# yyNoBug/VAE_segmentation

Hardware: AMD Instinct MI355X
Metric: 3D train-step volumes/sec at 96^3 batch=2 (joint VAE+seg) (higher is better)
Workload: dtype bf16; 1 GPU; configs[1]: 96^3 joint VAE+seg training step (joint_train), batch=2/GPU, bf16 activations + fp32 accumulate, SGD momentum 0.9, VAE frozen, HIP-graph replay; global_batch=2, parallelism=dp1, activation_recomputation=False, tail_in_graph=True, nranks=1, grad_exchange=none (1 rank)

## Files before the change

vae_segmentation_amd/csrc/conv_api.hip:

```cpp
#include <stdlib.h>
#include "igemm_dispatch.h"

int g1_dispatch_k3_f32(const G1Params& p, int ck, int mt, int epi, int tiles, int row_tiles, hipStream_t s);
int g1_dispatch_k3_bf16(const G1Params& p, int ck, int mt, int epi, int tiles, int row_tiles, hipStream_t s);
int g1_dispatch_k3_f16(const G1Params& p, int ck, int mt, int epi, int tiles, int row_tiles, hipStream_t s);
int g1_k3_fa_supported(const G1Params& p, int ck, int mt);
int k3tw_slab_count(int n, int d, int h, int w);
int k3x_ea_capacity(int n, int c, int m);
int k3b_ea_capacity(int n, int c, int m);
int k2s2_scatter8_launch(const G1Params& p, int dtype, hipStream_t stream);
int g1_dispatch_k3_x3(const G1Params& p, int ck, int mt, int epi, int tiles, int row_tiles, hipStream_t s);

extern "C" int vs_conv_k3_f32_limbs(int d, int h, int w, int c_in) {
    const int on = vs_cfg().f32_limbs;
    if (!on) return 0;
    const int small = vs_cfg().k3_small;
    if (small && c_in % 32 == 0 && c_in <= 1024 && (long long)(d + 2) * (h + 2) * (w + 2) <= 512) return 0;
    return 1;
}

static int dispatch_k3(const G1Params& p, int dtype, int ck, int mt, int epi, int tiles, int row_tiles, hipStream_t s) {
    if (dtype == VS_F32 && vs_conv_k3_f32_limbs(p.D, p.H, p.W, p.C)) {
        G1Params q = p;
        const int ckx = vs_k3x_ck(p.C);
        q.nch = p.C / ckx;
        const int rows16 = epi == EPI_SOFTMAX2 ? 16 : p.rb_total * 16;
        int mtx = 16;
        if (rows16 % 32 == 0 && (long long)tiles * (rows16 / 32) >= 256 && (ckx == 8 || (size_t)2 * p.N * (p.C + p.M) * sizeof(float) <= 3000)) mtx = 32;
        return g1_dispatch_k3_x3(q, ckx, mtx, epi, tiles, rows16 / mtx, s);
    }
    if (dtype == VS_F32) return g1_dispatch_k3_f32(p, ck, mt, epi, tiles, row_tiles, s);
    if (dtype == VS_BF16) return g1_dispatch_k3_bf16(p, ck, mt, epi, tiles, row_tiles, s);
    return g1_dispatch_k3_f16(p, ck, mt, epi, tiles, row_tiles, s);
}

static int pick_mt(int rows16, long long tiles) {
    const int min_wgs = vs_cfg().mt_min_wgs;
    const int cands[3] = {64, 32, 16};
    for (int i = 0; i < 3; ++i) {
        const int mt = cands[i];
        if (rows16 % mt) continue;
        if (tiles * (rows16 / mt) >= min_wgs || mt == 16) return mt;
    }
    return 16;
}

static int check_common(const void* x, const void* w, int n, int d, int h, int w_, int c_in, int dtype) {
    if (!x || !w) return VS_EINVAL;
    if (n <= 0 || d <= 0 || h <= 0 || w_ <= 0) return VS_ESHAPE;
    if (!(c_in == 8 || c_in == 16 || (c_in % 32 == 0 && c_in > 0 && c_in <= 256))) return VS_ESHAPE;
    if (!vs_dtype_ok(dtype)) return VS_EDTYPE;
    if (((uintptr_t)x & 15) || ((uintptr_t)w & 15)) return VS_EALIGN;
    if ((double)n * d * h * w_ * c_in >= 2147483648.0) return VS_ESHAPE;
    return VS_OK;
}

static inline long long g1_ea_capacity() { return 256; }

static int gather_impl(const void* x, const double* x_stats, const void* w_packed, const float* bias,
                       void* y, double* y_stats, const void* mask_x, const double* mask_stats, double* sums,
                       int n, int d, int h, int w, int c_in, int m_out, int kind, int dtype, float eps, void* stream,
                       const void* fa_x = nullptr, const double* fa_sums = nullptr, void* fa_dx = nullptr, int* fa_query = nullptr, float* wg_ws = nullptr,
                       unsigned int* ea_sync = nullptr, unsigned int* ea_fault = nullptr, int* ea_query = nullptr, const void* ea_add = nullptr) {
    int rc = check_common(x, w_packed, n, d, h, w, c_in, dtype);
    if (rc) return rc;
    if (!y || m_out <= 0 || m_out % 8 || ((uintptr_t)y & 15)) return VS_EINVAL;
    if (kind != VS_CONV_K3 && kind != VS_CONV_K2S2) return VS_EINVAL;
    if (kind == VS_CONV_K2S2 && ((d | h | w) & 1)) return VS_ESHAPE;
    G1Params p{};
    p.x = x; p.x_stats = x_stats; p.wp = w_packed; p.bias = bias; p.y = y; p.y_stats = y_stats; p.prob = nullptr;
    p.mask_x = mask_x; p.mask_stats = mask_stats; p.sums = sums;
    p.fa_x = fa_x; p.fa_sums = fa_sums; p.fa_dx = fa_dx; p.wg_ws = wg_ws;
    p.ea_sync = ea_sync; p.ea_fault = ea_fault; p.ea_add = ea_add;
    if (sums && (!mask_x || !mask_stats || y_stats)) return VS_EINVAL;
    p.N = n; p.D = d; p.H = h; p.W = w;
    p.C = c_in; p.M = m_out;
    p.rb_total = (m_out + 15) / 16;
    const int ck = c_in < 32 ? c_in : 32;
    p.nch = c_in / ck;
    p.eps = eps;
    p.inv_count_in = 1.0 / ((double)d * h * w);
    long long tiles;
    if (kind == VS_CONV_K3) {
        p.Do = d; p.Ho = h; p.Wo = w;
        p.tyn = (h + 3) / 4; p.txn = (w + 15) / 16;
        p.tiles_per_sample = ((d + 3) / 4) * p.tyn * p.txn;
    } else {
        p.Do = d / 2; p.Ho = h / 2; p.Wo = w / 2;
        p.tyn = p.txn = 0;
        p.tiles_per_sample = vs_ceil_div((long long)p.Do * p.Ho * p.Wo, 256);
        if (ck == 32 && p.nch >= 2 && (long long)p.tiles_per_sample * n * p.rb_total <= 64) {
            p.tiles_per_sample = vs_ceil_div((long long)p.Do * p.Ho * p.Wo, 64);
            p.tyn = 64;
        }
    }
    tiles = (long long)p.tiles_per_sample * n;
    p.inv_count_out = 1.0 / ((double)p.Do * p.Ho * p.Wo);
    const int rows16 = p.rb_total * 16;
    int mt = (kind != VS_CONV_K3 && p.tyn == 64) ? 16 : pick_mt(rows16, tiles);
    if (kind == VS_CONV_K3 && fa_x != nullptr && ck == 32 && mt == 16 && rows16 % 32 == 0) mt = 32;
    const int row_tiles = rows16 / mt;
    if (kind == VS_CONV_K2S2 && (ea_query != nullptr || ea_sync != nullptr)) {
        const bool ok = sums != nullptr && mt == 16 && tiles * row_tiles <= g1_ea_capacity();
        if (ea_query != nullptr) { *ea_query = ok ? 1 : 0; return VS_OK; }
        if (!ok) return VS_ESHAPE;
        p.ea_items = p.tiles_per_sample * row_tiles;
    }
    if (ea_query != nullptr) {
        *ea_query = (kind == VS_CONV_K3 && dtype != VS_F32 && ck == 32 && mt == 16 && sums != nullptr && !fa_x &&
                     !((long long)(d + 2) * (h + 2) * (w + 2) <= 512 && c_in <= 1024) && tiles * row_tiles <= k3b_ea_capacity(n, c_in, m_out)) ? 1 : 0;
        if (kind == VS_CONV_K3 && dtype == VS_F32 && sums != nullptr && !fa_x && vs_conv_k3_f32_limbs(d, h, w, c_in) && vs_k3x_ck(c_in) == 8 && c_in > 8) {
            const long long rows16 = p.rb_total;
            const bool mt32 = (p.rb_total * 16) % 32 == 0 && tiles * (p.rb_total / 2) >= 256;
            *ea_query = (!mt32 && tiles * rows16 <= k3x_ea_capacity(n, c_in, m_out)) ? 1 : 0;
        }
        return VS_OK;
    }
    if (fa_query != nullptr) {
        if (dtype == VS_F32)
            *fa_query = kind == VS_CONV_K3 && vs_conv_k3_f32_limbs(d, h, w, c_in) &&
                        ((c_in == 8 && m_out == 8 && n * 8 <= 192 && vs_k3x_toeplitz(8, 8, 27)) ||
                         (c_in == 16 && m_out == 16 && n * 16 <= 192 && vs_k3x_ck(16) == 8));
        else
            *fa_query = kind == VS_CONV_K3 ? g1_k3_fa_supported(p, ck, mt) : 0;
        return VS_OK;
    }
    if (kind == VS_CONV_K3) {
        return dispatch_k3(p, dtype, ck, mt, EPI_RAW, (int)tiles, row_tiles, (hipStream_t)stream);
    }
    return g1_dispatch_k2s2(p, dtype, ck, mt, (int)tiles, row_tiles, (hipStream_t)stream);
}

extern "C" int vs_conv_gather_fwd(const void* x, const double* x_stats, const void* w_packed, const float* bias,
                                  void* y, double* y_stats, int n, int d, int h, int w, int c_in, int m_out,
                                  int kind, int dtype, float eps, void* stream) {
    return gather_impl(x, x_stats, w_packed, bias, y, y_stats, nullptr, nullptr, nullptr, n, d, h, w, c_in, m_out, kind, dtype, eps, stream);
}

extern "C" int vs_conv_gather_bwd_data(const void* x, const void* w_packed, void* y, const void* mask_x,
                                       const double* mask_stats, double* sums, int n, int d, int h, int w, int c_in,
                                       int m_out, int kind, int dtype, float eps, void* stream) {
    if (!mask_x || !mask_stats || !sums) return VS_EINVAL;
    return gather_impl(x, nullptr, w_packed, nullptr, y, nullptr, mask_x, mask_stats, sums, n, d, h, w, c_in, m_out, kind, dtype, eps, stream);
}

extern "C" int vs_conv_k3_bwd_data_fused_apply(const void* g, const void* act_x, const double* act_stats, const double* act_sums,
                                               const void* w_packed, void* y, const void* mask_x, const double* mask_stats, double* sums,
                                               void* dx_out, int n, int d, int h, int w, int c_in, int m_out, int dtype, float eps,
                                               void* stream) {
    if (!g || !act_x || !act_stats || !act_sums) return VS_EINVAL;
    if ((mask_x == nullptr) != (sums == nullptr) || (mask_x == nullptr) != (mask_stats == nullptr)) return VS_EINVAL;
    if (dtype == VS_F32 && !vs_conv_k3_fused_apply_supported(n, d, h, w, c_in, m_out, mask_x != nullptr, dtype)) return VS_ESHAPE;
    if (((uintptr_t)act_x & 15) || (dx_out && ((uintptr_t)dx_out & 15))) return VS_EALIGN;
    return gather_impl(g, act_stats, w_packed, nullptr, y, nullptr, mask_x, mask_stats, sums, n, d, h, w, c_in, m_out, VS_CONV_K3, dtype, eps,
                       stream, act_x, act_sums, dx_out);
}

extern "C" int vs_conv_k3_fused_apply_supported(int n, int d, int h, int w, int c_in, int m_out, int lazy_input, int dtype) {
    if (!vs_dtype_ok(dtype)) return 0;
    static const char dummy[16] __attribute__((aligned(16))) = {0};
    static double dsink[2];
    int ok = 0;
    const int rc = gather_impl(dummy, (const double*)dummy, dummy, nullptr, (void*)dummy, nullptr, lazy_input ? dummy : nullptr,
                               lazy_input ? (const double*)dummy : nullptr, lazy_input ? dsink : nullptr, n, d, h, w, c_in, m_out, VS_CONV_K3,
                               dtype, 1e-5f, nullptr, dummy, (const double*)dummy, nullptr, &ok);
    return rc == VS_OK ? ok : 0;
}

extern "C" int vs_conv_k3_bwd_data_applied_supported(int n, int d, int h, int w, int c_in, int m_out, int dtype) {
    const int on = vs_cfg().epilogue_apply;
    if (!on || !vs_dtype_ok(dtype)) return 0;
    static const char dummy[16] __attribute__((aligned(16))) = {0};
    static double dsink[2];
    int ok = 0;
    const int rc = gather_impl(dummy, nullptr, dummy, nullptr, (void*)dummy, nullptr, dummy, (const double*)dummy, dsink, n, d, h, w, c_in, m_out, VS_CONV_K3, dtype,
                               1e-5f, nullptr, nullptr, nullptr, nullptr, nullptr, nullptr, nullptr, nullptr, &ok);
    return rc == VS_OK ? ok : 0;
}

extern "C" int vs_conv_k3_bwd_data_applied(const void* x, const void* w_packed, void* y, const void* mask_x, const double* mask_stats, double* sums,
                                           unsigned int* sync, unsigned int* fault, int n, int d, int h, int w, int c_in, int m_out, int dtype, float eps, void* stream) {
    if (!mask_x || !mask_stats || !sums || !sync || !fault) return VS_EINVAL;
    if (((uintptr_t)sync & 127) || ((uintptr_t)fault & 3)) return VS_EALIGN;
    if (!vs_conv_k3_bwd_data_applied_supported(n, d, h, w, c_in, m_out, dtype)) return VS_ESHAPE;
    return gather_impl(x, nullptr, w_packed, nullptr, y, nullptr, mask_x, mask_stats, sums, n, d, h, w, c_in, m_out, VS_CONV_K3, dtype, eps, stream,
                       nullptr, nullptr, nullptr, nullptr, nullptr, sync, fault);
}

extern "C" int vs_conv_k3_bwd_data_wgrad_supported(int n, int d, int h, int w, int c_in, int m_out, int dtype) {
    const int on = vs_cfg().fuse_wgrad;
    if (!on || (dtype != VS_BF16 && dtype != VS_F16)) return 0;
    if (c_in != 8 || m_out != 8 || n <= 0 || n * 8 > 192 || d <= 0 || h <= 0 || w <= 0) return 0;
    if ((double)n * d * h * w * 16 >= 2147483648.0) return 0;
    return vs_k3_toeplitz(8, 8, 27, dtype) ? 1 : 0;
}

extern "C" int vs_conv_k3_bwd_data_wgrad_slabs(int n, int d, int h, int w) {
    if (n <= 0 || d <= 0 || h <= 0 || w <= 0) return 0;
    return k3tw_slab_count(n, d, h, w);
}

extern "C" int vs_conv_k3_bwd_data_wgrad(const void* g, const void* act_x, const double* act_stats, const double* act_sums, const void* w_packed, void* y,
                                         const void* mask_x, const double* mask_stats, double* sums, float* slabs, int n, int d, int h, int w, int c_in,
                                         int m_out, int dtype, float eps, void* stream) {
    if (!g || !slabs || !mask_x || !mask_stats || !sums) return VS_EINVAL;
    if ((act_x == nullptr) != (act_stats == nullptr) || (act_x == nullptr) != (act_sums == nullptr)) return VS_EINVAL;
    if (!vs_conv_k3_bwd_data_wgrad_supported(n, d, h, w, c_in, m_out, dtype)) return VS_ESHAPE;
    if (((uintptr_t)slabs & 15) || (act_x && ((uintptr_t)act_x & 15))) return VS_EALIGN;
    return gather_impl(g, act_stats, w_packed, nullptr, y, nullptr, mask_x, mask_stats, sums, n, d, h, w, c_in, m_out, VS_CONV_K3, dtype, eps,
                       stream, act_x, act_sums, nullptr, nullptr, slabs);
}

extern "C" int vs_conv_k3_softmax2_bwd_data(const float* prob, const float* gprob, const void* gprob_cl, const void* w_packed, void* y, const void* mask_x,
                                            const double* mask_stats, double* sums, float* slabs, double* bias_part, int n, int d, int h, int w, int dtype,
                                            float eps, float drop_p, unsigned long long drop_seed, void* stream) {
    if (!prob || (!gprob && !gprob_cl) || !w_packed || !y || !mask_x || !mask_stats || !sums) return VS_EINVAL;
    if (bias_part && !slabs) return VS_EINVAL;
    if (!vs_conv_k3_bwd_data_wgrad_supported(n, d, h, w, 8, 8, dtype)) return VS_ESHAPE;
    if (((uintptr_t)w_packed & 15) || ((uintptr_t)y & 15) || ((uintptr_t)mask_x & 15) || (gprob_cl && ((uintptr_t)gprob_cl & 15)) || (slabs && ((uintptr_t)slabs & 15)) ||
        ((uintptr_t)prob & 3) || ((uintptr_t)gprob & 3)) return VS_EALIGN;
    if (!(drop_p >= 0.f && drop_p < 1.f)) return VS_EINVAL;
    G1Params p{};
    p.wp = w_packed; p.y = y; p.mask_x = mask_x; p.mask_stats = mask_stats; p.sums = sums;
    p.sm_prob = prob; p.sm_gprob = gprob; p.sm_gcl = gprob_cl; p.wg_ws = slabs; p.wg_bias = bias_part;
    p.drop_p = drop_p; p.drop_seed = drop_seed;
    p.N = n; p.D = d; p.H = h; p.W = w; p.Do = d; p.Ho = h; p.Wo = w; p.C = 8; p.M = 8; p.rb_total = 1; p.nch = 1;
    p.eps = eps;
    p.inv_count_in = 1.0 / ((double)d * h * w); p.inv_count_out = p.inv_count_in;
    return dispatch_k3(p, dtype, 8, 16, EPI_RAW, 0, 1, (hipStream_t)stream);
}

static int scatter_impl(const void* x, const double* x_stats, const void* w_packed, const float* bias, void* y,
                        const void* mask_x, const double* mask_stats, double* sums, int n, int d, int h, int w, int c_in,
                        int m_out, int dtype, float eps, void* stream,
                        unsigned int* ea_sync = nullptr, unsigned int* ea_fault = nullptr, int* ea_query = nullptr, const void* ea_add = nullptr) {
    int rc = check_common(x, w_packed, n, d, h, w, c_in, dtype);
    if (rc) return rc;
    if (!y || m_out <= 0 || m_out % 8 || ((uintptr_t)y & 15)) return VS_EINVAL;
    G1Params p{};
    p.x = x; p.x_stats = x_stats; p.wp = w_packed; p.bias = bias; p.y = y; p.y_stats = nullptr; p.prob = nullptr;
    p.mask_x = mask_x; p.mask_stats = mask_stats; p.sums = sums;
    p.inv_count_out = 1.0 / (8.0 * d * h * w);
    p.N = n; p.D = d; p.H = h; p.W = w;
    p.Do = d; p.Ho = h; p.Wo = w;
    p.C = c_in; p.M = m_out;
    p.rb_total = (8 * m_out + 15) / 16;
    const int ck = c_in < 32 ? c_in : 32;
    p.nch = c_in / ck;
    p.eps = eps;
    p.inv_count_in = 1.0 / ((double)d * h * w);
    p.tiles_per_sample = vs_ceil_div((long long)d * h * w, 256);
    const long long tiles = (long long)p.tiles_per_sample * n;
    const int stream8 = vs_cfg().k2s2_stream;
    const bool ea_asked = ea_query != nullptr || ea_sync != nullptr;
    if (!ea_asked && stream8 && sums && c_in == 8 && m_out == 8 && dtype != VS_F32 && !bias && !x_stats) {
        rc = k2s2_scatter8_launch(p, dtype, (hipStream_t)stream);
        if (rc != VS_ESHAPE) return rc;
    }
    const int rows16 = p.rb_total * 16;
    const int mt = pick_mt(rows16, tiles);
    if (ea_asked) {
        const bool ok = sums != nullptr && mt == 16 && tiles * (rows16 / mt) <= g1_ea_capacity();
        if (ea_query != nullptr) { *ea_query = ok ? 1 : 0; return VS_OK; }
        if (!ok) return VS_ESHAPE;
        p.ea_sync = ea_sync; p.ea_fault = ea_fault; p.ea_add = ea_add;
        p.ea_items = p.tiles_per_sample * (rows16 / mt);
    }
    return g1_dispatch_pw(p, dtype, ck, mt, (int)tiles, rows16 / mt, (hipStream_t)stream);
}

extern "C" int vs_conv_scatter_fwd(const void* x, const double* x_stats, const void* w_packed, const float* bias,
                                   void* y, int n, int d, int h, int w, int c_in, int m_out, int dtype, float eps,
                                   void* stream) {
    return scatter_impl(x, x_stats, w_packed, bias, y, nullptr, nullptr, nullptr, n, d, h, w, c_in, m_out, dtype, eps, stream);
}

extern "C" int vs_conv_scatter_bwd_data(const void* x, const void* w_packed, void* y, const void* mask_x,
                                        const double* mask_stats, double* sums, int n, int d, int h, int w, int c_in,
                                        int m_out, int dtype, float eps, void* stream) {
    if (!mask_x || !mask_stats || !sums) return VS_EINVAL;
    return scatter_impl(x, nullptr, w_packed, nullptr, y, mask_x, mask_stats, sums, n, d, h, w, c_in, m_out, dtype, eps, stream);
}

extern "C" int vs_conv_s2_bwd_data_applied_supported(int n, int d, int h, int w, int c_in, int m_out, int scatter, int dtype) {
    const int on = vs_cfg().epilogue_apply;
    if (!on || !vs_dtype_ok(dtype)) return 0;
    static const char dummy[16] __attribute__((aligned(16))) = {0};
    static double dsink[2];
    int ok = 0;
    const int rc = scatter ? scatter_impl(dummy, nullptr, dummy, nullptr, (void*)dummy, dummy, (const double*)dummy, dsink, n, d, h, w, c_in, m_out, dtype, 1e-5f, nullptr,
                                          nullptr, nullptr, &ok)
                           : gather_impl(dummy, nullptr, dummy, nullptr, (void*)dummy, nullptr, dummy, (const double*)dummy, dsink, n, d, h, w, c_in, m_out, VS_CONV_K2S2, dtype,
                                         1e-5f, nullptr, nullptr, nullptr, nullptr, nullptr, nullptr, nullptr, nullptr, &ok);
    return rc == VS_OK ? ok : 0;
}

extern "C" int vs_conv_s2_bwd_data_applied(const void* x, const void* w_packed, void* y, const void* mask_x, const double* mask_stats, double* sums, const void* add,
                                           unsigned int* sync, unsigned int* fault, int n, int d, int h, int w, int c_in, int m_out, int scatter, int dtype, float eps,
                                           void* stream) {
    if (!mask_x || !mask_stats || !sums || !sync || !fault) return VS_EINVAL;
    if (((uintptr_t)sync & 127) || ((uintptr_t)fault & 3) || (add && ((uintptr_t)add & 15))) return VS_EALIGN;
    if (!vs_conv_s2_bwd_data_applied_supported(n, d, h, w, c_in, m_out, scatter, dtype)) return VS_ESHAPE;
    if (scatter) return scatter_impl(x, nullptr, w_packed, nullptr, y, mask_x, mask_stats, sums, n, d, h, w, c_in, m_out, dtype, eps, stream, sync, fault, nullptr, add);
    return gather_impl(x, nullptr, w_packed, nullptr, y, nullptr, mask_x, mask_stats, sums, n, d, h, w, c_in, m_out, VS_CONV_K2S2, dtype, eps, stream,
                       nullptr, nullptr, nullptr, nullptr, nullptr, sync, fault, nullptr, add);
}

extern "C" int vs_conv_k3_softmax2_fwd(const void* x, const double* x_stats, const void* w_packed, const float* bias,
                                       float* prob, int n, int d, int h, int w, int c_in, int dtype, float eps,
                                       void* stream) {
    return vs_conv_k3_softmax2_dropout_fwd(x, x_stats, w_packed, bias, prob, n, d, h, w, c_in, dtype, eps, 0.f, 0ull, stream);
}

extern "C" int vs_conv_k3_softmax2_dropout_fwd(const void* x, const double* x_stats, const void* w_packed, const float* bias,
                                               float* prob, int n, int d, int h, int w, int c_in, int dtype, float eps,
                                               float drop_p, unsigned long long drop_seed, void* stream) {
    return vs_conv_k3_softmax2_cl_fwd(x, x_stats, w_packed, bias, prob, nullptr, n, d, h, w, c_in, dtype, eps, drop_p, drop_seed, stream);
}

extern "C" int vs_conv_k3_softmax2_cl_fwd(const void* x, const double* x_stats, const void* w_packed, const float* bias,
                                          float* prob, void* prob_cl, int n, int d, int h, int w, int c_in, int dtype, float eps,
                                          float drop_p, unsigned long long drop_seed, void* stream) {
    if (drop_p < 0.f || drop_p >= 1.f) return VS_EINVAL;
    if (prob_cl && dtype == VS_F32) return VS_EDTYPE;
    if (prob_cl && ((uintptr_t)prob_cl & 15)) return VS_EALIGN;
    int rc = check_common(x, w_packed, n, d, h, w, c_in, dtype);
    if (rc) return rc;
    if (!prob || c_in != 8) return VS_ESHAPE;
    G1Params p{};
    p.x = x; p.x_stats = x_stats; p.wp = w_packed; p.bias = bias; p.y = prob_cl; p.y_stats = nullptr; p.prob = prob;
    p.mask_x = nullptr; p.mask_stats = nullptr; p.sums = nullptr; p.inv_count_out = 1.0 / ((double)d * h * w);
    p.drop_p = drop_p; p.drop_seed = drop_seed;
    p.N = n; p.D = d; p.H = h; p.W = w;
    p.Do = d; p.Ho = h; p.Wo = w;
    p.C = c_in; p.M = 8;
    p.rb_total = 1;
    p.nch = 1;
    p.eps = eps;
    p.inv_count_in = 1.0 / ((double)d * h * w);
    p.tyn = (h + 3) / 4; p.txn = (w + 15) / 16;
    p.tiles_per_sample = ((d + 3) / 4) * p.tyn * p.txn;
    const long long tiles = (long long)p.tiles_per_sample * n;
    return dispatch_k3(p, dtype, 8, 16, EPI_SOFTMAX2, (int)tiles, 1, (hipStream_t)stream);
}
```

vae_segmentation_amd/csrc/igemm_k3_bf16.hip:

```cpp
#define VS_CHAIN_STAMPS_TU 1
#include "igemm_k3_h16.inc"

int g1_dispatch_k3_bf16(const G1Params& p, int ck, int mt, int epi, int tiles, int row_tiles, hipStream_t s) {
    return dispatch_k3_h16<unsigned short>(p, ck, mt, epi, tiles, row_tiles, s);
}

int g1_k3_fa_supported(const G1Params& p, int ck, int mt) { return k3_h16_fa_supported(p, ck, mt) ? 1 : 0; }
int k3tw_slab_count(int n, int d, int h, int w) { return k3tw_grid(n, d, h, w); }

int chain_dispatch_k3s_bf16(const K3Chain& c, int bwd, hipStream_t s) { return k3s_chain_launch<unsigned short>(c, bwd != 0, s); }
int k3b_ea_capacity(int n, int c, int m) { return k3b_ea_max_wgs(n, c, m); }
```

vae_segmentation_amd/csrc/igemm_k3_f16.hip:

```cpp
#undef VS_STAMPS
#undef VS_STAMPS_LITE
#include "igemm_k3_h16.inc"

int g1_dispatch_k3_f16(const G1Params& p, int ck, int mt, int epi, int tiles, int row_tiles, hipStream_t s) {
    return dispatch_k3_h16<vs_half>(p, ck, mt, epi, tiles, row_tiles, s);
}

int chain_dispatch_k3s_f16(const K3Chain& c, int bwd, hipStream_t s) { return k3s_chain_launch<vs_half>(c, bwd != 0, s); }
```

vae_segmentation_amd/csrc/igemm_k3_h16.inc:

```
#include "igemm_dispatch.h"
#include "igemm_k3b.h"
#include "igemm_k3t.h"
#include "igemm_k3s.h"
#include "igemm_k3tw.h"

#define K3B_CASE(CKV, MTV)                                                                              \
    if (ck == CKV && mt == MTV)                                                                          \
        return p.sums ? k3b_launch<T, CKV, MTV, EPI_RAW, true>(p, tiles, row_tiles, s)                   \
                      : k3b_launch<T, CKV, MTV, EPI_RAW, false>(p, tiles, row_tiles, s);

static inline bool k3_h16_fa_supported(const G1Params& p, int ck, int mt) {
    if (ck == 32) return false;
    if (ck == 8 && p.C == 8 && p.M == 8) return true;
    const bool lazy_in = p.sums != nullptr;
    if (mt == 16 && k3b_use_tall(p)) return ck == 16;
    if (mt == 64) mt = 32;
    return (ck == 16 && mt == 16) || (ck == 8 && mt == 16 && !lazy_in) || (ck == 16 && mt == 32 && !lazy_in);
}

template <typename T>
static int dispatch_k3_h16(const G1Params& p, int ck, int mt, int epi, int tiles, int row_tiles, hipStream_t s) {
    if (p.fa_x != nullptr && (epi != EPI_RAW || !k3_h16_fa_supported(p, ck, mt))) return VS_ESHAPE;
    if (p.wg_ws != nullptr || p.sm_prob != nullptr) {
        if (!(ck == 8 && p.C == 8 && p.M == 8 && epi == EPI_RAW && p.sums)) return VS_ESHAPE;
        return k3tw_launch<T>(p, s);
    }
    const bool short_tiles = vs_cfg().k3_short_tiles && ck == 32 && mt == 16 && epi == EPI_RAW && !p.fa_x && !k3s_takes(p, ck) &&
                             (long long)tiles * row_tiles <= 128 && (long long)p.N * ((p.D + 3) / 4) * ((p.H + 1) / 2) * p.txn * row_tiles <= 256;
    const bool shorter_tiles = short_tiles && vs_cfg().k3_short_tiles >= 2 &&
                               (long long)p.N * ((p.D + 3) / 4) * ((p.H + 1) / 2) * p.txn * row_tiles <= 128 && (long long)p.N * ((p.D + 3) / 4) * p.H * p.txn * row_tiles <= 256;
    if (p.ea_sync != nullptr) {
        if (!(ck == 32 && mt == 16 && epi == EPI_RAW && p.sums && !p.fa_x) || k3s_takes(p, ck)) return VS_ESHAPE;
        if (shorter_tiles) return k3b_launch_t<T, 32, 16, EPI_RAW, true, 1, false, false, true>(p, tiles, row_tiles, s);
        if (short_tiles) return k3b_launch_t<T, 32, 16, EPI_RAW, true, 2, false, false, true>(p, tiles, row_tiles, s);
        return k3b_launch_t<T, 32, 16, EPI_RAW, true, 4, false, false, true>(p, tiles, row_tiles, s);
    }
    if (ck == 8 && p.C == 8 && p.M == 8) {
        if (epi == EPI_SOFTMAX2) return k3t_launch<T, EPI_SOFTMAX2, false, 8>(p, s);
        return p.sums ? k3t_launch<T, EPI_RAW, true, 8>(p, s) : k3t_launch<T, EPI_RAW, false, 8>(p, s);
    }
    if (epi == EPI_RAW && k3s_takes(p, ck))
        return p.sums ? k3s_launch<T, true>(p, s) : k3s_launch<T, false>(p, s);
    const bool tall = mt == 16 && ck < 32 && k3b_use_tall(p);
    if (epi == EPI_SOFTMAX2) return VS_ESHAPE;
    if (tall) {
        if (ck == 8) return p.sums ? k3b_launch<T, 8, 16, EPI_RAW, true, 8>(p, tiles, row_tiles, s) : k3b_launch<T, 8, 16, EPI_RAW, false, 8>(p, tiles, row_tiles, s);
        return p.sums ? k3b_launch<T, 16, 16, EPI_RAW, true, 8>(p, tiles, row_tiles, s) : k3b_launch<T, 16, 16, EPI_RAW, false, 8>(p, tiles, row_tiles, s);
    }
    if (shorter_tiles) return p.sums ? k3b_launch<T, 32, 16, EPI_RAW, true, 1>(p, tiles, row_tiles, s) : k3b_launch<T, 32, 16, EPI_RAW, false, 1>(p, tiles, row_tiles, s);
    if (short_tiles) return p.sums ? k3b_launch<T, 32, 16, EPI_RAW, true, 2>(p, tiles, row_tiles, s) : k3b_launch<T, 32, 16, EPI_RAW, false, 2>(p, tiles, row_tiles, s);
    if (mt == 64) { mt = 32; row_tiles *= 2; }
    K3B_CASE(8, 16) K3B_CASE(8, 32) K3B_CASE(16, 16) K3B_CASE(16, 32) K3B_CASE(32, 16) K3B_CASE(32, 32)
    return VS_ESHAPE;
}
```

vae_segmentation_amd/csrc/igemm_k3b.h:

```cpp
#pragma once
#include <stdlib.h>
#include "igemm.h"
#include "chain.h"

#ifdef VS_STAMPS
__device__ unsigned long long g_k3_stamps[2048 * 8];
extern "C" int vs_debug_read_k3_stamps(unsigned long long* host, int n) {
    return (int)hipMemcpyFromSymbol(host, HIP_SYMBOL(g_k3_stamps), sizeof(unsigned long long) * n);
}
#define K3_TICK(i) do { const unsigned long long now_ = __builtin_amdgcn_s_memtime(); tk_acc[i] += now_ - tk_last; tk_last = now_; } while (0)
#define K3_TICK_INIT unsigned long long tk_acc[8] = {0, 0, 0, 0, 0, 0, 0, 0}; unsigned long long tk_last = __builtin_amdgcn_s_memtime(); tk_acc[7] = __builtin_amdgcn_s_memrealtime();
#define K3_TICK_FLUSH do { if (threadIdx.x == 0) { tk_acc[7] = (tk_acc[7] << 32) | (__builtin_amdgcn_s_memrealtime() & 0xffffffffull); for (int i_ = 0; i_ < 8; ++i_) g_k3_stamps[((blockIdx.y * gridDim.x + blockIdx.x) & 2047) * 8 + i_] = tk_acc[i_]; } } while (0)
#elif defined(VS_STAMPS_LITE)
__device__ unsigned long long g_k3_stamps[2048 * 8];
extern "C" int vs_debug_read_k3_stamps(unsigned long long* host, int n) {
    return (int)hipMemcpyFromSymbol(host, HIP_SYMBOL(g_k3_stamps), sizeof(unsigned long long) * n);
}
#define K3_TICK(i)
#define K3_TICK_INIT const unsigned long long tk_rt0 = __builtin_amdgcn_s_memrealtime();
#define K3_TICK_FLUSH do { if (threadIdx.x == 0) { unsigned long long* d_ = g_k3_stamps + ((blockIdx.y * gridDim.x + blockIdx.x) & 2047) * 8; d_[0] = 1; d_[7] = (tk_rt0 << 32) | (__builtin_amdgcn_s_memrealtime() & 0xffffffffull); } } while (0)
#else
#define K3_TICK(i)
#define K3_TICK_INIT
#define K3_TICK_FLUSH
#endif

#define K3B_LDS_RED 0
#define K3B_LDS_TAPS 2048
#define K3B_LDS_TILE 2304

template <int CK, int MT, int YT = 4>
struct K3BGeom {
    static constexpr int RB = MT / 16;
    static constexpr int TV = 6 * (YT + 2) * 18;
    static constexpr bool SMALLC = CK < 32;
    static constexpr int NKGC = SMALLC ? (27 * CK + 31) / 32 : 27;
    static constexpr int CKB = CK * 2;
    static constexpr int TILE_BYTES = ((TV * (CKB / 16) + 255) / 256) * 256 * 16;
    static constexpr int NWF = RB * NKGC * 64;
    static constexpr int W_BYTES = ((NWF + 255) / 256) * 256 * 16;
};

template <int CK, int MT, int EPI, bool SUMS, int YT = 4, bool HS = false, typename T = unsigned short, bool FA = false, bool EA = false>
__global__ __launch_bounds__(256) __attribute__((amdgpu_waves_per_eu(
    YT == 8 ? 2 : (CK == 32 ? ((MT == 32 || FA) ? 1 : 2) : (MT == 32 ? (SUMS ? 2 : 3) : ((CK == 16 && SUMS) || FA ? 3 : 4))), 8))) void k3b_kernel(const G1Params p) {
    K3_TICK_INIT
    using GEO = K3BGeom<CK, MT, YT>;
    static_assert(!FA || (!HS && EPI == EPI_RAW), "fused apply: backward-data kernels");
    static_assert(!EA || (SUMS && !FA && !HS && EPI == EPI_RAW), "epilogue apply: backward-data kernels with fused sums");
    static_assert(YT == 4 || (YT == 8 && CK < 32 && MT == 16) || ((YT == 2 || YT == 1) && CK == 32 && MT == 16), "tall tiles: single-chunk layers, 16 rows; short tiles: 32-channel chunks, 16 rows");
    constexpr int TV = GEO::TV, PLANE = (YT + 2) * 18;
    static_assert(CK == 8 || CK == 16 || CK == 32, "chunk width");
    constexpr int RB = GEO::RB, NKGC = GEO::NKGC, CKB = GEO::CKB, NWF = GEO::NWF;
    constexpr bool SMALLC = GEO::SMALLC;
    constexpr int U = CKB / 16;
    constexpr int NU = TV * U;
    constexpr int NIT = (NU + 255) / 256;
    constexpr int NWI = (NWF + 255) / 256;
    extern __shared__ __attribute__((aligned(16))) char smem[];
    float* s_red = (float*)(smem + K3B_LDS_RED);
    int* s_taps = (int*)(smem + K3B_LDS_TAPS);
    char* s_tile = smem + K3B_LDS_TILE;
    char* s_w = s_tile + GEO::TILE_BYTES;
    float* s_scale = (float*)(s_w + GEO::W_BYTES);
    float* s_shift = s_scale + p.N * p.C;
    float* s_mkm = s_shift + p.N * p.C;
    float* s_mkr = s_mkm + p.N * p.M;
    float* s_fa = s_shift + p.N * p.C + (SUMS ? 2 * p.N * p.M : 0);

    const int tid = threadIdx.x, lane = tid & 63, wave = tid >> 6, col = lane & 15, g = lane >> 4;
    const int rb0 = blockIdx.y * RB;
    constexpr bool has_stats = HS;
    constexpr bool has_sums = SUMS;
    const int total_tiles = p.tiles_per_sample * p.N;
    const i32x4 xrsrc = make_rsrc(p.x, (unsigned int)((long long)p.N * p.D * p.H * p.W * p.C * 2));
    const i32x4 frsrc = make_rsrc(FA ? p.fa_x : p.x, (unsigned int)((long long)p.N * p.D * p.H * p.W * p.C * 2));
    const i32x4 dxrsrc = make_rsrc(FA && p.fa_dx != nullptr ? p.fa_dx : p.x, (FA && p.fa_dx != nullptr) ? (unsigned int)((long long)p.N * p.D * p.H * p.W * p.C * 2) : 0u);
    const u32x4* __restrict__ wp = (const u32x4*)p.wp;

    const double* st_src = SUMS ? p.mask_stats : p.x_stats;
    const int st_n = SUMS ? p.N * p.M : (has_stats ? p.N * p.C : 0);
    double st_pre[2] = {0.0, 1.0};
    if (tid < st_n) stat_load(st_src, (size_t)tid, (size_t)st_n, st_pre);
    double fa_pre[2][2] = {{0.0, 1.0}, {0.0, 0.0}};
    if constexpr (FA) {
        if (tid >= 64 && tid < 64 + p.N * p.C) {
            stat_load(p.x_stats, (size_t)(tid - 64), (size_t)p.N * p.C, fa_pre[0]);
            stat_load(p.fa_sums, (size_t)(tid - 64), (size_t)p.N * p.C, fa_pre[1]);
        }
    }

    const int part = tid % U;
    int rel_off[NIT], tzyx[NIT];
    const int lds_w0 = (tid / U) * CKB;
    unsigned int swzbits = 0, cbits = 0;
#pragma unroll
    for (int b = 0; b < NIT; ++b) {
        const int u = tid + b * 256;
        const int tv = u / U;
        const int tx_ = tv % 18, ty_ = (tv / 18) % (YT + 2), tz_ = tv / PLANE;
        cbits |= (u < NU && tz_ >= 1 && tz_ <= 4 && ty_ >= 1 && ty_ <= YT && tx_ >= 1 && tx_ <= 16) ? (1u << b) : 0u;
        rel_off[b] = (((tz_ * p.H + ty_) * p.W + tx_) * p.C + part * 8) * 2;
        tzyx[b] = u < NU ? (tz_ | (ty_ << 8) | (tx_ << 16)) : 0x00ffffff;
        if (CK == 32) swzbits |= (unsigned int)((tx_ >> 2) & 1) << b;
    }
    int w_off[NWI];
#pragma unroll
    for (int i = 0; i < NWI; ++i) {
        int f = tid + i * 256;
        if (f > NWF - 1) f = NWF - 1;
        const int rb = f / (NKGC * 64), r = f - rb * (NKGC * 64);
        w_off[i] = (rb0 + rb) * (p.nch * NKGC * 64) + r;
    }

    u32x4 xv[NIT], wv[NWI], fv[FA ? NIT : 1];
    unsigned int okbits = 0;
    struct Coord { int n, z0, y0, x0; };
    auto tile_coord = [&](int t) {
        Coord c;
        c.n = fdiv(t, p.fd_m[0], p.fd_s[0]);
        const int tl = t - c.n * p.tiles_per_sample;
        const int tz = fdiv(tl, p.fd_m[1], p.fd_s[1]);
        const int r = tl - tz * (p.txn * p.tyn);
        const int ty = fdiv(r, p.fd_m[2], p.fd_s[2]);
        c.z0 = tz * 4; c.y0 = ty * YT; c.x0 = (r - ty * p.txn) * 16;
        return c;
    };
    auto load_w = [&](int ch) {
#pragma unroll
        for (int i = 0; i < NWI; ++i) wv[i] = wp[w_off[i] + ch * (NKGC * 64)];
    };
    auto load_x = [&](const Coord& c, int ch) {
        const int n = c.n, z0 = c.z0, y0 = c.y0, x0 = c.x0;
        const int base = ((((n * p.D + z0 - 1) * p.H + y0 - 1) * p.W + x0 - 1) * p.C + ch * CK) * 2;
        okbits = 0;
#pragma unroll
        for (int b = 0; b < NIT; ++b) {
            const int gz = z0 - 1 + (tzyx[b] & 0xff), gy = y0 - 1 + ((tzyx[b] >> 8) & 0xff), gx = x0 - 1 + (tzyx[b] >> 16);
            const bool ok = (unsigned)gz < (unsigned)p.D && (unsigned)gy < (unsigned)p.H && (unsigned)gx < (unsigned)p.W;
            okbits |= ok ? (1u << b) : 0u;
            xv[b] = __builtin_bit_cast(u32x4, vs_raw_buffer_load_b128(xrsrc, ok ? base + rel_off[b] : -1, 0, 0));
            if constexpr (FA) fv[b] = __builtin_bit_cast(u32x4, vs_raw_buffer_load_b128(frsrc, ok ? base + rel_off[b] : -1, 0, 0));
        }
    };
    auto write_x_fa = [&](const Coord& c, int ch) {
        f32x2 r2[4], s2[4], a2[4], b2[4];
        const int c0 = c.n * p.C + ch * CK + part * 8;
#pragma unroll
        for (int i = 0; i < 4; ++i) {
            r2[i] = *(const f32x2*)(s_fa + 0 * p.N * p.C + c0 + 2 * i);
            s2[i] = *(const f32x2*)(s_fa + 1 * p.N * p.C + c0 + 2 * i);
            a2[i] = *(const f32x2*)(s_fa + 2 * p.N * p.C + c0 + 2 * i);
            b2[i] = *(const f32x2*)(s_fa + 3 * p.N * p.C + c0 + 2 * i);
        }
        const int base = ((((c.n * p.D + c.z0 - 1) * p.H + c.y0 - 1) * p.W + c.x0 - 1) * p.C + ch * CK) * 2;
        const bool store_dx = p.fa_dx != nullptr && blockIdx.y == 0;
#pragma unroll
        for (int b = 0; b < NIT; ++b) {
            u32x4 v;
#pragma unroll
            for (int i = 0; i < 4; ++i) {
                f32x2 g2, x2;
                g2[0] = H16<T>::lo(xv[b][i]); g2[1] = H16<T>::hi(xv[b][i]);
                x2[0] = H16<T>::lo(fv[b][i]); x2[1] = H16<T>::hi(fv[b][i]);
                const f32x2 xh = x2 * r2[i] + s2[i];
                f32x2 gm;
                gm[0] = xh[0] > 0.f ? g2[0] : 0.f;
                gm[1] = xh[1] > 0.f ? g2[1] : 0.f;
                const f32x2 d = r2[i] * (gm - a2[i] - xh * b2[i]);
                v[i] = H16<T>::pack2(d);
            }
            const bool ok = (okbits >> b) & 1u;
#pragma unroll
            for (int i = 0; i < 4; ++i) v[i] = ok ? v[i] : 0u;
            const int pw = CK == 32 ? (part ^ (int)(((swzbits >> b) & 1u) << 1)) : part;
            *(u32x4*)(s_tile + lds_w0 + b * 4096 + pw * 16) = v;
            if (store_dx)
                vs_raw_buffer_store_b128(__builtin_bit_cast(i32x4, v), dxrsrc, (ok && ((cbits >> b) & 1u)) ? base + rel_off[b] : -1, 0, 0);
        }
    };
    auto write_x = [&](int n, int ch) {
        f32x2 sc[4], sh[4];
        if (has_stats) {
            const int c0 = n * p.C + ch * CK + part * 8;
#pragma unroll
            for (int i = 0; i < 4; ++i) {
                sc[i] = *(const f32x2*)(s_scale + c0 + 2 * i);
                sh[i] = *(const f32x2*)(s_shift + c0 + 2 * i);
            }
        }
#pragma unroll
        for (int b = 0; b < NIT; ++b) {
            u32x4 v = xv[b];
            if (has_stats) {
                const u32x4 a = act8<T>(v, sc, sh);
                const bool ok = (okbits >> b) & 1u;
#pragma unroll
                for (int i = 0; i < 4; ++i) v[i] = ok ? a[i] : 0u;
            }
            const int pw = CK == 32 ? (part ^ (int)(((swzbits >> b) & 1u) << 1)) : part;
            *(u32x4*)(s_tile + lds_w0 + b * 4096 + pw * 16) = v;
        }
    };
    auto write_w = [&]() {
#pragma unroll
        for (int i = 0; i < NWI; ++i)
            *(u32x4*)(s_w + (tid + i * 256) * 16) = wv[i];
    };

    int t, t_end, G;
    if (((int)gridDim.x & 7) == 0) {
        const int xcd = (int)blockIdx.x & 7;
        G = (int)gridDim.x >> 3;
        t = (int)(((long long)total_tiles * xcd) >> 3) + ((int)blockIdx.x >> 3);
        t_end = (int)(((long long)total_tiles * (xcd + 1)) >> 3);
    } else { G = (int)gridDim.x; t = (int)blockIdx.x; t_end = total_tiles; }
    Coord cur = tile_coord(t), nxt = cur;
    load_w(0);
    load_x(cur, 0);
    float bv[RB][4];
#pragma unroll
    for (int rb = 0; rb < RB; ++rb)
#pragma unroll
        for (int r = 0; r < 4; ++r) {
            const int row = (rb0 + rb) * 16 + 4 * g + r;
            bv[rb][r] = (p.bias != nullptr && row < (EPI == EPI_SOFTMAX2 ? 2 : p.M)) ? p.bias[row] : 0.f;
        }
    const i32x4 yrsrc = make_rsrc(p.y, (unsigned int)((long long)p.N * p.D * p.H * p.W * p.M * 2));
    const i32x4 mrsrc = make_rsrc(p.mask_x, (unsigned int)((long long)p.N * p.D * p.H * p.W * p.M * 2));
    for (int i = tid; i < st_n; i += 256) {
        double st[2] = {st_pre[0], st_pre[1]};
        if (i != tid) stat_load(st_src, (size_t)i, (size_t)st_n, st);
        float m, r;
        stats_to_mean_rstd_fast(st, SUMS ? p.inv_count_out : p.inv_count_in, p.eps, m, r);
        if constexpr (SUMS) { s_mkm[i] = m; s_mkr[i] = r; }
        else { s_scale[i] = r; s_shift[i] = -m * r; }
    }
    if constexpr (FA) {
        if (tid >= 64 && tid < 64 + p.N * p.C) {
            const int i = tid - 64;
            float m, r;
            stats_to_mean_rstd_fast(fa_pre[0], p.inv_count_in, p.eps, m, r);
            s_fa[0 * p.N * p.C + i] = r;
            s_fa[1 * p.N * p.C + i] = -m * r;
            s_fa[2 * p.N * p.C + i] = (float)(fa_pre[1][0] * p.inv_count_in);
            s_fa[3 * p.N * p.C + i] = (float)(fa_pre[1][1] * p.inv_count_in);
        }
    }

    int baddr[3];
    if constexpr (SMALLC) {
        if (tid < NKGC * 4) {
            int tap = (tid >> 2) * (32 / CK) + ((tid & 3) * 8) / CK;
            if (tap > 26) tap = 13;
            const int dz = tap / 9, dy = (tap / 3) % 3, dx = tap % 3;
            s_taps[tid] = (dz * PLANE + dy * 18 + dx) * CKB + (((tid & 3) * 8) % CK) * 2;
        }
        baddr[0] = (wave * PLANE + col) * CKB;
    } else {
#pragma unroll
        for (int dx = 0; dx < 3; ++dx) baddr[dx] = (wave * PLANE + col) * CKB + ((g ^ ((((col + dx) >> 2) & 1) << 1)) * 16);
    }
    const char* s_wl = s_w + lane * 16;

    float ssum[RB][4], ssq[RB][4];
#pragma unroll
    for (int rb = 0; rb < RB; ++rb)
#pragma unroll
        for (int r = 0; r < 4; ++r) { ssum[rb][r] = 0.f; ssq[rb][r] = 0.f; }

#pragma unroll
    for (int rb = 0; rb < RB; ++rb)
#pragma unroll
        for (int r = 0; r < 4; ++r) asm volatile("" : "+v"(bv[rb][r]));
    constexpr bool restage_w = !SMALLC;
    bool first = true;
    if constexpr (SMALLC) write_w();
    __syncthreads();
    K3_TICK(0);

    for (; t < t_end; t += G) {
        const int n = cur.n, z0 = cur.z0, y0 = cur.y0, x0 = cur.x0;
        const int oz = z0 + wave;
        const int ebase = ((((n * p.D + oz) * p.H + y0) * p.W + x0 + col) * p.M + rb0 * 16 + 4 * g) * 2;
        const bool zx_ok = oz < p.D && x0 + col < p.W;
        f32x4 acc[RB][YT];
#pragma unroll
        for (int rb = 0; rb < RB; ++rb)
#pragma unroll
            for (int cg = 0; cg < YT; ++cg) acc[rb][cg] = f32x4{0.f, 0.f, 0.f, 0.f};
        u32x2 mk[RB][YT];
        i32x2 pkk[EA ? RB : 1][EA ? YT : 1];

        for (int ch = 0; ch < p.nch; ++ch) {
            if (!first) __syncthreads();
            K3_TICK(1);
            if constexpr (FA) write_x_fa(cur, ch); else write_x(n, ch);
            if constexpr (restage_w) write_w();
            first = false;
            K3_TICK(2);
            __syncthreads();
            K3_TICK(3);
            const bool last_ch = ch + 1 == p.nch;
            if constexpr (EPI == EPI_RAW) {
                if (has_sums && last_ch) {
#pragma unroll
                    for (int rb = 0; rb < RB; ++rb)
#pragma unroll
                        for (int cg = 0; cg < YT; ++cg) {
                            const bool valid = zx_ok && y0 + cg < p.H && (rb0 + rb) * 16 + 4 * g < p.M;
                            mk[rb][cg] = __builtin_bit_cast(u32x2, vs_raw_buffer_load_b64(mrsrc, valid ? ebase + cg * p.W * p.M * 2 + rb * 32 : -1, 0, 0));
                        }
                }
            }
            {
                const int tn = last_ch ? t + G : t;
                if (last_ch) nxt = tile_coord(tn);
                if (tn < t_end) {
                    if constexpr (restage_w) load_w(last_ch ? 0 : ch + 1);
                    load_x(last_ch ? nxt : cur, last_ch ? 0 : ch + 1);
                }
            }

            K3_TICK(4);
            auto read_kg = [&](int kg, u32x4 (&a)[RB], u32x4 (&b)[YT]) {
#pragma unroll
                for (int rb = 0; rb < RB; ++rb) a[rb] = *(const u32x4*)(s_wl + (rb * NKGC + kg) * 1024);
                if constexpr (SMALLC) {
                    const int o = baddr[0] + s_taps[kg * 4 + g];
#pragma unroll
                    for (int cg = 0; cg < YT; ++cg) b[cg] = *(const u32x4*)(s_tile + o + cg * 18 * CKB);
                } else {
                    const int dz = kg / 9, dy = (kg / 3) % 3, dx = kg % 3;
#pragma unroll
                    for (int cg = 0; cg < YT; ++cg) b[cg] = *(const u32x4*)(s_tile + baddr[dx] + ((dz * PLANE + (dy + cg) * 18 + dx) * CKB));
                }
            };
            u32x4 fa[2][RB], fb[2][YT];
            read_kg(0, fa[0], fb[0]);
#pragma unroll
            for (int kg = 0; kg < NKGC; ++kg) {
                if (kg + 1 < NKGC) read_kg(kg + 1, fa[(kg + 1) & 1], fb[(kg + 1) & 1]);
#pragma unroll
                for (int rb = 0; rb < RB; ++rb)
#pragma unroll
                    for (int cg = 0; cg < YT; ++cg) acc[rb][cg] = mfma16(fa[kg & 1][rb], fb[kg & 1][cg], acc[rb][cg], (T*)nullptr);
                __builtin_amdgcn_sched_barrier(0);
            }
        }

        K3_TICK(5);
        if constexpr (EPI == EPI_SOFTMAX2) {
            if (g == 0) {
                const float b0 = bv[0][0], b1 = bv[0][1];
                const size_t V = (size_t)p.D * p.H * p.W;
#pragma unroll
                for (int cg = 0; cg < YT; ++cg) {
                    const int oy = y0 + cg, ox = x0 + col;
                    if (!(oz < p.D && oy < p.H && ox < p.W)) continue;
                    float l0 = acc[0][cg][0] + b0, l1 = acc[0][cg][1] + b1;
                    const size_t v = ((size_t)oz * p.H + oy) * p.W + ox;
                    if (p.drop_p > 0.f) {
                        l0 *= dropout_scale(p.drop_seed, ((unsigned long long)n * 2 + 0) * V + v, p.drop_p);
                        l1 *= dropout_scale(p.drop_seed, ((unsigned long long)n * 2 + 1) * V + v, p.drop_p);
                    }
                    const float mx = fmaxf(l0, l1);
                    const float e0 = __expf(l0 - mx), e1 = __expf(l1 - mx);
                    const float inv = 1.f / (e0 + e1);
                    p.prob[((size_t)n * 2 + 0) * V + v] = e0 * inv;
                    p.prob[((size_t)n * 2 + 1) * V + v] = e1 * inv;
                }
            }
        } else {
#pragma unroll
            for (int rb = 0; rb < RB; ++rb) {
                const bool rvalid = (rb0 + rb) * 16 + 4 * g < p.M;
                float mm[4] = {0.f, 0.f, 0.f, 0.f}, mr[4] = {0.f, 0.f, 0.f, 0.f};
                if (has_sums && rvalid) {
                    const int row = (rb0 + rb) * 16 + 4 * g;
#pragma unroll
                    for (int r = 0; r < 4; ++r) { mm[r] = s_mkm[n * p.M + row + r]; mr[r] = s_mkr[n * p.M + row + r]; }
                }
#pragma unroll
                for (int cg = 0; cg < YT; ++cg) {
                    const bool valid = rvalid && zx_ok && y0 + cg < p.H;
                    f32x2 lo, hi;
                    lo[0] = acc[rb][cg][0] + bv[rb][0]; lo[1] = acc[rb][cg][1] + bv[rb][1];
                    hi[0] = acc[rb][cg][2] + bv[rb][2]; hi[1] = acc[rb][cg][3] + bv[rb][3];
                    i32x2 pk;
                    pk[0] = (int)H16<T>::pack2(lo);
                    pk[1] = (int)H16<T>::pack2(hi);
                    if constexpr (EA) pkk[rb][cg] = pk;
                    else vs_raw_buffer_store_b64(pk, yrsrc, valid ? ebase + cg * p.W * p.M * 2 + rb * 32 : -1, 0, 0);
                    float v[4];
                    v[0] = H16<T>::lo((unsigned int)pk[0]); v[1] = H16<T>::hi((unsigned int)pk[0]);
                    v[2] = H16<T>::lo((unsigned int)pk[1]); v[3] = H16<T>::hi((unsigned int)pk[1]);
                    if (!valid) { v[0] = 0.f; v[1] = 0.f; v[2] = 0.f; v[3] = 0.f; }
                    if (has_sums) {
                        const u32x2 xx = mk[rb][cg];
                        float xv4[4];
                        xv4[0] = H16<T>::lo(xx[0]); xv4[1] = H16<T>::hi(xx[0]);
                        xv4[2] = H16<T>::lo(xx[1]); xv4[3] = H16<T>::hi(xx[1]);
#pragma unroll
                        for (int r = 0; r < 4; ++r) {
                            const float xh = (xv4[r] - mm[r]) * mr[r];
                            const float gm = xh > 0.f ? v[r] : 0.f;
                            ssum[rb][r] += gm; ssq[rb][r] += gm * xh;
                        }
                    } else {
#pragma unroll
                        for (int r = 0; r < 4; ++r) { ssum[rb][r] += v[r]; ssq[rb][r] += v[r] * v[r]; }
                    }
                }
            }
            double* const red_dst0 = has_sums ? p.sums : p.y_stats;
            double* const red_dst = red_dst0;
            if (red_dst != nullptr) {
                const bool flush = t + G >= t_end || nxt.n != n;
                if (flush) {
#pragma unroll
                    for (int rb = 0; rb < RB; ++rb)
#pragma unroll
                        for (int r = 0; r < 4; ++r) {
                            float s = ssum[rb][r], q = ssq[rb][r];
                            { s = row16_sum(s); q = row16_sum(q); }
                            if (col == 0) {
                                const int lr = rb * 16 + 4 * g + r;
                                s_red[(wave * 64 + lr) * 2 + 0] = s;
                                s_red[(wave * 64 + lr) * 2 + 1] = q;
                            }
                            ssum[rb][r] = 0.f; ssq[rb][r] = 0.f;
                        }
                    __syncthreads();
                    if (tid < MT * 2) {
                        const int lr = tid >> 1, st = tid & 1;
                        const int row = rb0 * 16 + lr;
                        if (row < p.M) {
                            const double tot = (double)s_red[(0 * 64 + lr) * 2 + st] + (double)s_red[(1 * 64 + lr) * 2 + st] +
                                               (double)s_red[(2 * 64 + lr) * 2 + st] + (double)s_red[(3 * 64 + lr) * 2 + st];
                            stat_add(red_dst, (size_t)n * p.M + row, (size_t)p.N * p.M, st, tot);
                        }
                    }
                    if (t + G < t_end) __syncthreads();
                }
            }
            if constexpr (EA) {
                unsigned int* ctr = p.ea_sync + (size_t)n * 256;
                chain_arrive8(ctr);
                chain_wait8(ctr, (unsigned int)p.ea_items, p.ea_fault);
                if (tid < MT) {
                    const int row = rb0 * 16 + tid;
                    float m = 0.f, r = 1.f, a = 0.f, b = 0.f;
                    if (row < p.M) {
                        stats_to_mean_rstd(p.mask_stats, (size_t)n * p.M + row, (size_t)p.N * p.M, p.inv_count_out, p.eps, m, r);
                        double sv[2];
                        stat_load_sc1(p.sums, (size_t)n * p.M + row, (size_t)p.N * p.M, sv);
                        a = (float)(sv[0] * p.inv_count_out);
                        b = (float)(sv[1] * p.inv_count_out);
                    }
                    *(f32x4*)(s_red + tid * 4) = f32x4{m, r, a, b};
                }
                __syncthreads();
#pragma unroll
                for (int rb = 0; rb < RB; ++rb) {
                    const bool rvalid = (rb0 + rb) * 16 + 4 * g < p.M;
                    f32x4 tb[4];
#pragma unroll
                    for (int r = 0; r < 4; ++r) tb[r] = *(const f32x4*)(s_red + (rb * 16 + 4 * g + r) * 4);
#pragma unroll
                    for (int cg = 0; cg < YT; ++cg) {
                        const bool valid = rvalid && zx_ok && y0 + cg < p.H;
                        const unsigned int gw[2] = {(unsigned int)pkk[rb][cg][0], (unsigned int)pkk[rb][cg][1]};
                        const u32x2 xx = mk[rb][cg];
                        const float gv[4] = {H16<T>::lo(gw[0]), H16<T>::hi(gw[0]), H16<T>::lo(gw[1]), H16<T>::hi(gw[1])};
                        const float xq[4] = {H16<T>::lo(xx[0]), H16<T>::hi(xx[0]), H16<T>::lo(xx[1]), H16<T>::hi(xx[1])};
                        float o[4];
#pragma unroll
                        for (int r = 0; r < 4; ++r) {
                            o[r] = vs_in_bwd_apply1(gv[r], xq[r], tb[r][0], tb[r][1], tb[r][2], tb[r][3]);
                        }
                        i32x2 po;
                        po[0] = (int)H16<T>::pack2(f32x2{o[0], o[1]});
                        po[1] = (int)H16<T>::pack2(f32x2{o[2], o[3]});
                        vs_raw_buffer_store_b64(po, yrsrc, valid ? ebase + cg * p.W * p.M * 2 + rb * 32 : -1, 0, 0);
                    }
                }
            }
        }
        cur = nxt;
        K3_TICK(6);
    }
    K3_TICK_FLUSH;
}

static inline int k3b_ea_max_wgs(int n, int c, int m) {
    using GEO = K3BGeom<32, 16, 4>;
    const size_t lds = K3B_LDS_TILE + (size_t)GEO::TILE_BYTES + GEO::W_BYTES + (size_t)2 * n * c * sizeof(float) + (size_t)2 * n * m * sizeof(float);
    return 2 * (lds + 1024) <= 160 * 1024 ? 512 : 256;
}

static inline void k3b_fastdiv(int d, unsigned int& m, unsigned int& s) {
    s = 0;
    while ((1ll << s) < d) ++s;
    m = (unsigned int)((((1ull << (32 + s)) + (unsigned long long)d - 1) / (unsigned long long)d) - (1ull << 32));
}

template <typename T, int CK, int MT, int EPI, bool SUMS, int YT, bool HS, bool FA = false, bool EA = false>
static int k3b_launch_t(const G1Params& p_in, int tiles_total, int row_tiles, hipStream_t stream) {
    using GEO = K3BGeom<CK, MT, YT>;
    if (FA && (p_in.N * p_in.C > 192 || (CK < 32 && p_in.nch != 1) || !p_in.x_stats || !p_in.fa_sums)) return VS_ESHAPE;
    const size_t tables = (size_t)(FA ? 6 : 2) * p_in.N * p_in.C * sizeof(float) + (p_in.sums ? (size_t)2 * p_in.N * p_in.M * sizeof(float) : 0);
    const size_t lds = K3B_LDS_TILE + (size_t)GEO::TILE_BYTES + GEO::W_BYTES + tables;
    if (lds > 160 * 1024) return VS_ESHAPE;
    G1Params p = p_in;
    if (YT != 4) {
        p.tyn = (p.H + YT - 1) / YT;
        p.tiles_per_sample = ((p.D + 3) / 4) * p.tyn * p.txn;
        tiles_total = p.tiles_per_sample * p.N;
    }
    if ((long long)p.N * p.D * p.H * p.W * p.C * 2 >= 2147483648ll || (long long)p.N * p.D * p.H * p.W * p.M * 2 >= 2147483648ll) return VS_ESHAPE;
    k3b_fastdiv(p.tiles_per_sample, p.fd_m[0], p.fd_s[0]);
    k3b_fastdiv(p.txn * p.tyn, p.fd_m[1], p.fd_s[1]);
    k3b_fastdiv(p.txn, p.fd_m[2], p.fd_s[2]);
    if (SUMS != (p.sums != nullptr) || (SUMS && !FA && p.x_stats != nullptr)) return VS_EINVAL;
    auto kern = k3b_kernel<CK, MT, EPI, SUMS, YT, HS, T, FA, EA>;
    static const hipError_t attr_err =
        hipFuncSetAttribute((const void*)kern, hipFuncAttributeMaxDynamicSharedMemorySize, 160 * 1024);
    if (attr_err != hipSuccess) return (int)attr_err;
    const int per_cu = vs_cfg().k3_wgs_per_cu > 0 ? vs_cfg().k3_wgs_per_cu : 3;
    int wg = 256 * per_cu / (row_tiles < per_cu ? row_tiles : per_cu);
    if (wg < 256) wg = 256;
    const int gx = tiles_total < wg ? tiles_total : wg;
    if (EA) {
        if (gx != tiles_total || (long long)tiles_total * row_tiles > k3b_ea_max_wgs(p.N, p.C, p.M) || !p.ea_sync || !p.ea_fault) return VS_ESHAPE;
        p.ea_items = p.tiles_per_sample * row_tiles;
    }
    hipLaunchKernelGGL(kern, dim3(gx, row_tiles), dim3(256), lds, stream, p);
    VS_CHECK_LAUNCH();
    return VS_OK;
}

template <int CK, int MT, int EPI, bool SUMS, int YT>
constexpr bool k3b_has_fa() {
    return EPI == EPI_RAW && ((CK == 16 && MT == 16) || (CK == 8 && MT == 16 && !SUMS && YT == 4) || (CK == 16 && MT == 32 && !SUMS && YT == 4));
}

template <typename T, int CK, int MT, int EPI, bool SUMS, int YT = 4>
static int k3b_launch(const G1Params& p, int tiles_total, int row_tiles, hipStream_t stream) {
    if (p.fa_x != nullptr) {
        if constexpr (k3b_has_fa<CK, MT, EPI, SUMS, YT>()) return k3b_launch_t<T, CK, MT, EPI, SUMS, YT, false, true>(p, tiles_total, row_tiles, stream);
        else return VS_ESHAPE;
    }
    if (!SUMS && p.x_stats != nullptr) return k3b_launch_t<T, CK, MT, EPI, SUMS, YT, !SUMS>(p, tiles_total, row_tiles, stream);
    return k3b_launch_t<T, CK, MT, EPI, SUMS, YT, false>(p, tiles_total, row_tiles, stream);
}

static inline bool k3b_use_tall(const G1Params& p) {
    const int force = vs_cfg().k3_tall;
    if (force >= 0) return force != 0;
    const long long tall = (long long)((p.D + 3) / 4) * ((p.H + 7) / 8) * p.txn * p.N;
    return tall >= 256 && (long long)p.tiles_per_sample * p.N <= 2048;
}
```

Measured before the change: 898.3 volumes/s.

## Add eight-wave k3b variants splitting columns or row pairs for small grids

```diff
diff --git a/vae_segmentation_amd/csrc/conv_api.hip b/vae_segmentation_amd/csrc/conv_api.hip
--- a/vae_segmentation_amd/csrc/conv_api.hip
+++ b/vae_segmentation_amd/csrc/conv_api.hip
@@ -7,7 +7,8 @@
 int g1_k3_fa_supported(const G1Params& p, int ck, int mt);
 int k3tw_slab_count(int n, int d, int h, int w);
 int k3x_ea_capacity(int n, int c, int m);
-int k3b_ea_capacity(int n, int c, int m);
+int g1_k3_ea_supported_bf16(const G1Params& p, int ck, int mt, int tiles, int row_tiles);
+int g1_k3_ea_supported_f16(const G1Params& p, int ck, int mt, int tiles, int row_tiles);
 int k2s2_scatter8_launch(const G1Params& p, int dtype, hipStream_t stream);
 int g1_dispatch_k3_x3(const G1Params& p, int ck, int mt, int epi, int tiles, int row_tiles, hipStream_t s);
 
@@ -107,8 +108,9 @@
         p.ea_items = p.tiles_per_sample * row_tiles;
     }
     if (ea_query != nullptr) {
-        *ea_query = (kind == VS_CONV_K3 && dtype != VS_F32 && ck == 32 && mt == 16 && sums != nullptr && !fa_x &&
-                     !((long long)(d + 2) * (h + 2) * (w + 2) <= 512 && c_in <= 1024) && tiles * row_tiles <= k3b_ea_capacity(n, c_in, m_out)) ? 1 : 0;
+        *ea_query = 0;
+        if (kind == VS_CONV_K3 && dtype == VS_BF16) *ea_query = g1_k3_ea_supported_bf16(p, ck, mt, (int)tiles, row_tiles);
+        if (kind == VS_CONV_K3 && dtype == VS_F16) *ea_query = g1_k3_ea_supported_f16(p, ck, mt, (int)tiles, row_tiles);
         if (kind == VS_CONV_K3 && dtype == VS_F32 && sums != nullptr && !fa_x && vs_conv_k3_f32_limbs(d, h, w, c_in) && vs_k3x_ck(c_in) == 8 && c_in > 8) {
             const long long rows16 = p.rb_total;
             const bool mt32 = (p.rb_total * 16) % 32 == 0 && tiles * (p.rb_total / 2) >= 256;
diff --git a/vae_segmentation_amd/csrc/igemm_k3_bf16.hip b/vae_segmentation_amd/csrc/igemm_k3_bf16.hip
--- a/vae_segmentation_amd/csrc/igemm_k3_bf16.hip
+++ b/vae_segmentation_amd/csrc/igemm_k3_bf16.hip
@@ -9,4 +9,4 @@
 int k3tw_slab_count(int n, int d, int h, int w) { return k3tw_grid(n, d, h, w); }
 
 int chain_dispatch_k3s_bf16(const K3Chain& c, int bwd, hipStream_t s) { return k3s_chain_launch<unsigned short>(c, bwd != 0, s); }
-int k3b_ea_capacity(int n, int c, int m) { return k3b_ea_max_wgs(n, c, m); }
+int g1_k3_ea_supported_bf16(const G1Params& p, int ck, int mt, int tiles, int row_tiles) { return k3_h16_ea_supported<unsigned short>(p, ck, mt, tiles, row_tiles) ? 1 : 0; }
diff --git a/vae_segmentation_amd/csrc/igemm_k3_f16.hip b/vae_segmentation_amd/csrc/igemm_k3_f16.hip
--- a/vae_segmentation_amd/csrc/igemm_k3_f16.hip
+++ b/vae_segmentation_amd/csrc/igemm_k3_f16.hip
@@ -6,4 +6,6 @@
     return dispatch_k3_h16<vs_half>(p, ck, mt, epi, tiles, row_tiles, s);
 }
 
+int g1_k3_ea_supported_f16(const G1Params& p, int ck, int mt, int tiles, int row_tiles) { return k3_h16_ea_supported<vs_half>(p, ck, mt, tiles, row_tiles) ? 1 : 0; }
+
 int chain_dispatch_k3s_f16(const K3Chain& c, int bwd, hipStream_t s) { return k3s_chain_launch<vs_half>(c, bwd != 0, s); }
diff --git a/vae_segmentation_amd/csrc/igemm_k3_h16.inc b/vae_segmentation_amd/csrc/igemm_k3_h16.inc
--- a/vae_segmentation_amd/csrc/igemm_k3_h16.inc
+++ b/vae_segmentation_amd/csrc/igemm_k3_h16.inc
@@ -18,6 +18,42 @@
     return (ck == 16 && mt == 16) || (ck == 8 && mt == 16 && !lazy_in) || (ck == 16 && mt == 32 && !lazy_in);
 }
 
+static inline int k3b32_yt(const G1Params& p, long long tiles, int row_tiles) {
+    const int on = vs_cfg().k3_short_tiles;
+    const long long t2 = (long long)p.N * ((p.D + 3) / 4) * ((p.H + 1) / 2) * p.txn, t1 = (long long)p.N * ((p.D + 3) / 4) * p.H * p.txn;
+    if (!on || tiles * row_tiles > 128 || t2 * row_tiles > 256) return 4;
+    if (on >= 2 && t2 * row_tiles <= 128 && t1 * row_tiles <= 256) return 1;
+    return 2;
+}
+
+template <typename T, bool SUMS, bool HS, bool EA, int YT>
+static int k3b32_plan(const G1Params& p, int tiles, int row_tiles, hipStream_t s, bool dry) {
+    if constexpr (YT == 1) {
+        return k3b_launch_t<T, 32, 16, EPI_RAW, SUMS, YT, HS, false, EA, 4, K3B_WAVES4>(p, tiles, row_tiles, s, dry);
+    } else {
+        const long long grid4 = (long long)p.N * ((p.D + 3) / 4) * ((p.H + YT - 1) / YT) * p.txn * row_tiles;
+        const int cap = K3bInst<T, 32, 16, EPI_RAW, true, YT, false, false, true, 8, K3B_COLS>::capacity(p);
+        if (grid4 < cap) return k3b_launch_t<T, 32, 16, EPI_RAW, SUMS, YT, HS, false, EA, 8, K3B_COLS>(p, tiles, row_tiles, s, dry);
+        if (row_tiles % 2 == 0 && grid4 > cap && grid4 / 2 <= cap) return k3b_launch_t<T, 32, 16, EPI_RAW, SUMS, YT, HS, false, EA, 8, K3B_ROWS>(p, tiles, row_tiles, s, dry);
+        return k3b_launch_t<T, 32, 16, EPI_RAW, SUMS, YT, HS, false, EA, 4, K3B_WAVES4>(p, tiles, row_tiles, s, dry);
+    }
+}
+
+template <typename T, bool SUMS, bool HS, bool EA>
+static int k3b32_launch(const G1Params& p, int tiles, int row_tiles, hipStream_t s, bool dry) {
+    switch (k3b32_yt(p, tiles, row_tiles)) {
+        case 1: return k3b32_plan<T, SUMS, HS, EA, 1>(p, tiles, row_tiles, s, dry);
+        case 2: return k3b32_plan<T, SUMS, HS, EA, 2>(p, tiles, row_tiles, s, dry);
+        default: return k3b32_plan<T, SUMS, HS, EA, 4>(p, tiles, row_tiles, s, dry);
+    }
+}
+
+template <typename T>
+static bool k3_h16_ea_supported(const G1Params& p, int ck, int mt, int tiles, int row_tiles) {
+    if (!(ck == 32 && mt == 16 && p.sums && !p.fa_x) || k3s_takes(p, ck)) return false;
+    return k3b32_launch<T, true, false, true>(p, tiles, row_tiles, nullptr, true) == VS_OK;
+}
+
 template <typename T>
 static int dispatch_k3_h16(const G1Params& p, int ck, int mt, int epi, int tiles, int row_tiles, hipStream_t s) {
     if (p.fa_x != nullptr && (epi != EPI_RAW || !k3_h16_fa_supported(p, ck, mt))) return VS_ESHAPE;
@@ -25,15 +61,9 @@
         if (!(ck == 8 && p.C == 8 && p.M == 8 && epi == EPI_RAW && p.sums)) return VS_ESHAPE;
         return k3tw_launch<T>(p, s);
     }
-    const bool short_tiles = vs_cfg().k3_short_tiles && ck == 32 && mt == 16 && epi == EPI_RAW && !p.fa_x && !k3s_takes(p, ck) &&
-                             (long long)tiles * row_tiles <= 128 && (long long)p.N * ((p.D + 3) / 4) * ((p.H + 1) / 2) * p.txn * row_tiles <= 256;
-    const bool shorter_tiles = short_tiles && vs_cfg().k3_short_tiles >= 2 &&
-                               (long long)p.N * ((p.D + 3) / 4) * ((p.H + 1) / 2) * p.txn * row_tiles <= 128 && (long long)p.N * ((p.D + 3) / 4) * p.H * p.txn * row_tiles <= 256;
     if (p.ea_sync != nullptr) {
         if (!(ck == 32 && mt == 16 && epi == EPI_RAW && p.sums && !p.fa_x) || k3s_takes(p, ck)) return VS_ESHAPE;
-        if (shorter_tiles) return k3b_launch_t<T, 32, 16, EPI_RAW, true, 1, false, false, true>(p, tiles, row_tiles, s);
-        if (short_tiles) return k3b_launch_t<T, 32, 16, EPI_RAW, true, 2, false, false, true>(p, tiles, row_tiles, s);
-        return k3b_launch_t<T, 32, 16, EPI_RAW, true, 4, false, false, true>(p, tiles, row_tiles, s);
+        return k3b32_launch<T, true, false, true>(p, tiles, row_tiles, s, false);
     }
     if (ck == 8 && p.C == 8 && p.M == 8) {
         if (epi == EPI_SOFTMAX2) return k3t_launch<T, EPI_SOFTMAX2, false, 8>(p, s);
@@ -47,9 +77,12 @@
         if (ck == 8) return p.sums ? k3b_launch<T, 8, 16, EPI_RAW, true, 8>(p, tiles, row_tiles, s) : k3b_launch<T, 8, 16, EPI_RAW, false, 8>(p, tiles, row_tiles, s);
         return p.sums ? k3b_launch<T, 16, 16, EPI_RAW, true, 8>(p, tiles, row_tiles, s) : k3b_launch<T, 16, 16, EPI_RAW, false, 8>(p, tiles, row_tiles, s);
     }
-    if (shorter_tiles) return p.sums ? k3b_launch<T, 32, 16, EPI_RAW, true, 1>(p, tiles, row_tiles, s) : k3b_launch<T, 32, 16, EPI_RAW, false, 1>(p, tiles, row_tiles, s);
-    if (short_tiles) return p.sums ? k3b_launch<T, 32, 16, EPI_RAW, true, 2>(p, tiles, row_tiles, s) : k3b_launch<T, 32, 16, EPI_RAW, false, 2>(p, tiles, row_tiles, s);
+    if (ck == 32 && mt == 16) {
+        if (p.sums) return k3b32_launch<T, true, false, false>(p, tiles, row_tiles, s, false);
+        if (p.x_stats) return k3b32_launch<T, false, true, false>(p, tiles, row_tiles, s, false);
+        return k3b32_launch<T, false, false, false>(p, tiles, row_tiles, s, false);
+    }
     if (mt == 64) { mt = 32; row_tiles *= 2; }
-    K3B_CASE(8, 16) K3B_CASE(8, 32) K3B_CASE(16, 16) K3B_CASE(16, 32) K3B_CASE(32, 16) K3B_CASE(32, 32)
+    K3B_CASE(8, 16) K3B_CASE(8, 32) K3B_CASE(16, 16) K3B_CASE(16, 32) K3B_CASE(32, 32)
     return VS_ESHAPE;
 }
diff --git a/vae_segmentation_amd/csrc/igemm_k3b.h b/vae_segmentation_amd/csrc/igemm_k3b.h
--- a/vae_segmentation_amd/csrc/igemm_k3b.h
+++ b/vae_segmentation_amd/csrc/igemm_k3b.h
@@ -1,5 +1,6 @@
 #pragma once
 #include <stdlib.h>
+#include <mutex>
 #include "igemm.h"
 #include "chain.h"
 
@@ -29,23 +30,31 @@
 #define K3B_LDS_TAPS 2048
 #define K3B_LDS_TILE 2304
 
-template <int CK, int MT, int YT = 4>
+template <int CK, int MT, int YT = 4, int NT = 256, int RBX = 1, bool XS = false>
 struct K3BGeom {
     static constexpr int RB = MT / 16;
     static constexpr int TV = 6 * (YT + 2) * 18;
     static constexpr bool SMALLC = CK < 32;
     static constexpr int NKGC = SMALLC ? (27 * CK + 31) / 32 : 27;
     static constexpr int CKB = CK * 2;
-    static constexpr int TILE_BYTES = ((TV * (CKB / 16) + 255) / 256) * 256 * 16;
-    static constexpr int NWF = RB * NKGC * 64;
-    static constexpr int W_BYTES = ((NWF + 255) / 256) * 256 * 16;
+    static constexpr int TILE_BYTES = ((TV * (CKB / 16) + NT - 1) / NT) * NT * 16;
+    static constexpr int NWF = RBX * RB * NKGC * 64;
+    static constexpr int W_BYTES = ((NWF + NT - 1) / NT) * NT * 16;
+    static constexpr int XS_BYTES = XS ? 4 * RB * (YT / 2) * 4 * 2 * 64 * 4 : 0;
 };
 
-template <int CK, int MT, int EPI, bool SUMS, int YT = 4, bool HS = false, typename T = unsigned short, bool FA = false, bool EA = false>
-__global__ __launch_bounds__(256) __attribute__((amdgpu_waves_per_eu(
+#define K3B_WAVES4 0
+#define K3B_COLS 1
+#define K3B_ROWS 2
+template <int CK, int MT, int EPI, bool SUMS, int YT = 4, bool HS = false, typename T = unsigned short, bool FA = false, bool EA = false, int NW = 4, int SPL = K3B_WAVES4>
+__global__ __launch_bounds__(NW * 64) __attribute__((amdgpu_waves_per_eu(
     YT == 8 ? 2 : (CK == 32 ? ((MT == 32 || FA) ? 1 : 2) : (MT == 32 ? (SUMS ? 2 : 3) : ((CK == 16 && SUMS) || FA ? 3 : 4))), 8))) void k3b_kernel(const G1Params p) {
     K3_TICK_INIT
-    using GEO = K3BGeom<CK, MT, YT>;
+    constexpr int NT = NW * 64;
+    constexpr bool CSPLIT = SPL == K3B_COLS, RPAIR = SPL == K3B_ROWS;
+    static_assert(NW == 4 ? SPL == K3B_WAVES4 : (NW == 8 && SPL != K3B_WAVES4 && CK == 32 && MT == 16 && !FA && EPI == EPI_RAW && YT <= 4 && (!CSPLIT || YT >= 2)),
+                  "eight waves: the 32-channel chunks, 16 rows, no fused apply");
+    using GEO = K3BGeom<CK, MT, YT, NT, RPAIR ? 2 : 1, CSPLIT>;
     static_assert(!FA || (!HS && EPI == EPI_RAW), "fused apply: backward-data kernels");
     static_assert(!EA || (SUMS && !FA && !HS && EPI == EPI_RAW), "epilogue apply: backward-data kernels with fused sums");
     static_assert(YT == 4 || (YT == 8 && CK < 32 && MT == 16) || ((YT == 2 || YT == 1) && CK == 32 && MT == 16), "tall tiles: single-chunk layers, 16 rows; short tiles: 32-channel chunks, 16 rows");
@@ -55,21 +64,27 @@
     constexpr bool SMALLC = GEO::SMALLC;
     constexpr int U = CKB / 16;
     constexpr int NU = TV * U;
-    constexpr int NIT = (NU + 255) / 256;
-    constexpr int NWI = (NWF + 255) / 256;
+    constexpr int NIT = (NU + NT - 1) / NT;
+    constexpr int NWI = (NWF + NT - 1) / NT;
+    constexpr int MTW = RPAIR ? 2 * MT : MT;
+    constexpr int RS = NW == 8 ? 32 : 64;
+    constexpr int NE = CSPLIT ? YT / 2 : YT;
     extern __shared__ __attribute__((aligned(16))) char smem[];
     float* s_red = (float*)(smem + K3B_LDS_RED);
     int* s_taps = (int*)(smem + K3B_LDS_TAPS);
     char* s_tile = smem + K3B_LDS_TILE;
     char* s_w = s_tile + GEO::TILE_BYTES;
-    float* s_scale = (float*)(s_w + GEO::W_BYTES);
+    float* s_scale = (float*)(s_w + GEO::W_BYTES + GEO::XS_BYTES);
     float* s_shift = s_scale + p.N * p.C;
     float* s_mkm = s_shift + p.N * p.C;
     float* s_mkr = s_mkm + p.N * p.M;
     float* s_fa = s_shift + p.N * p.C + (SUMS ? 2 * p.N * p.M : 0);
 
     const int tid = threadIdx.x, lane = tid & 63, wave = tid >> 6, col = lane & 15, g = lane >> 4;
-    const int rb0 = blockIdx.y * RB;
+    const int wz = wave & 3;
+    const int q = NW == 8 ? __builtin_amdgcn_readfirstlane(tid >> 8) : 0;
+    const int rb0 = blockIdx.y * RB * (RPAIR ? 2 : 1);
+    const int rbw = rb0 + (RPAIR ? q * RB : 0);
     constexpr bool has_stats = HS;
     constexpr bool has_sums = SUMS;
     const int total_tiles = p.tiles_per_sample * p.N;
@@ -96,7 +111,7 @@
     unsigned int swzbits = 0, cbits = 0;
 #pragma unroll
     for (int b = 0; b < NIT; ++b) {
-        const int u = tid + b * 256;
+        const int u = tid + b * NT;
         const int tv = u / U;
         const int tx_ = tv % 18, ty_ = (tv / 18) % (YT + 2), tz_ = tv / PLANE;
         cbits |= (u < NU && tz_ >= 1 && tz_ <= 4 && ty_ >= 1 && ty_ <= YT && tx_ >= 1 && tx_ <= 16) ? (1u << b) : 0u;
@@ -107,7 +122,7 @@
     int w_off[NWI];
 #pragma unroll
     for (int i = 0; i < NWI; ++i) {
-        int f = tid + i * 256;
+        int f = tid + i * NT;
         if (f > NWF - 1) f = NWF - 1;
         const int rb = f / (NKGC * 64), r = f - rb * (NKGC * 64);
         w_off[i] = (rb0 + rb) * (p.nch * NKGC * 64) + r;
@@ -174,7 +189,7 @@
 #pragma unroll
             for (int i = 0; i < 4; ++i) v[i] = ok ? v[i] : 0u;
             const int pw = CK == 32 ? (part ^ (int)(((swzbits >> b) & 1u) << 1)) : part;
-            *(u32x4*)(s_tile + lds_w0 + b * 4096 + pw * 16) = v;
+            *(u32x4*)(s_tile + lds_w0 + b * NT * 16 + pw * 16) = v;
             if (store_dx)
                 vs_raw_buffer_store_b128(__builtin_bit_cast(i32x4, v), dxrsrc, (ok && ((cbits >> b) & 1u)) ? base + rel_off[b] : -1, 0, 0);
         }
@@ -199,13 +214,13 @@
                 for (int i = 0; i < 4; ++i) v[i] = ok ? a[i] : 0u;
             }
             const int pw = CK == 32 ? (part ^ (int)(((swzbits >> b) & 1u) << 1)) : part;
-            *(u32x4*)(s_tile + lds_w0 + b * 4096 + pw * 16) = v;
+            *(u32x4*)(s_tile + lds_w0 + b * NT * 16 + pw * 16) = v;
         }
     };
     auto write_w = [&]() {
 #pragma unroll
         for (int i = 0; i < NWI; ++i)
-            *(u32x4*)(s_w + (tid + i * 256) * 16) = wv[i];
+            *(u32x4*)(s_w + (tid + i * NT) * 16) = wv[i];
     };
 
     int t, t_end, G;
@@ -223,12 +238,12 @@
     for (int rb = 0; rb < RB; ++rb)
 #pragma unroll
         for (int r = 0; r < 4; ++r) {
-            const int row = (rb0 + rb) * 16 + 4 * g + r;
+            const int row = (rbw + rb) * 16 + 4 * g + r;
             bv[rb][r] = (p.bias != nullptr && row < (EPI == EPI_SOFTMAX2 ? 2 : p.M)) ? p.bias[row] : 0.f;
         }
     const i32x4 yrsrc = make_rsrc(p.y, (unsigned int)((long long)p.N * p.D * p.H * p.W * p.M * 2));
     const i32x4 mrsrc = make_rsrc(p.mask_x, (unsigned int)((long long)p.N * p.D * p.H * p.W * p.M * 2));
-    for (int i = tid; i < st_n; i += 256) {
+    for (int i = tid; i < st_n; i += NT) {
         double st[2] = {st_pre[0], st_pre[1]};
         if (i != tid) stat_load(st_src, (size_t)i, (size_t)st_n, st);
         float m, r;
@@ -256,12 +271,12 @@
             const int dz = tap / 9, dy = (tap / 3) % 3, dx = tap % 3;
             s_taps[tid] = (dz * PLANE + dy * 18 + dx) * CKB + (((tid & 3) * 8) % CK) * 2;
         }
-        baddr[0] = (wave * PLANE + col) * CKB;
+        baddr[0] = (wz * PLANE + col) * CKB;
     } else {
 #pragma unroll
-        for (int dx = 0; dx < 3; ++dx) baddr[dx] = (wave * PLANE + col) * CKB + ((g ^ ((((col + dx) >> 2) & 1) << 1)) * 16);
-    }
-    const char* s_wl = s_w + lane * 16;
+        for (int dx = 0; dx < 3; ++dx) baddr[dx] = (wz * PLANE + (CSPLIT ? q * NE * 18 : 0) + col) * CKB + ((g ^ ((((col + dx) >> 2) & 1) << 1)) * 16);
+    }
+    const char* s_wl = s_w + lane * 16 + (RPAIR ? q * RB * NKGC * 1024 : 0);
 
     float ssum[RB][4], ssq[RB][4];
 #pragma unroll
@@ -281,16 +296,17 @@
 
     for (; t < t_end; t += G) {
         const int n = cur.n, z0 = cur.z0, y0 = cur.y0, x0 = cur.x0;
-        const int oz = z0 + wave;
-        const int ebase = ((((n * p.D + oz) * p.H + y0) * p.W + x0 + col) * p.M + rb0 * 16 + 4 * g) * 2;
+        const int oz = z0 + wz;
+        const int ebase = ((((n * p.D + oz) * p.H + y0) * p.W + x0 + col) * p.M + rbw * 16 + 4 * g) * 2;
         const bool zx_ok = oz < p.D && x0 + col < p.W;
-        f32x4 acc[RB][YT];
+        const int cgo = CSPLIT ? q * NE : 0;
+        f32x4 acc[RB][NE];
 #pragma unroll
         for (int rb = 0; rb < RB; ++rb)
 #pragma unroll
-            for (int cg = 0; cg < YT; ++cg) acc[rb][cg] = f32x4{0.f, 0.f, 0.f, 0.f};
-        u32x2 mk[RB][YT];
-        i32x2 pkk[EA ? RB : 1][EA ? YT : 1];
+            for (int cg = 0; cg < NE; ++cg) acc[rb][cg] = f32x4{0.f, 0.f, 0.f, 0.f};
+        u32x2 mk[RB][NE];
+        i32x2 pkk[EA ? RB : 1][EA ? NE : 1];
 
         for (int ch = 0; ch < p.nch; ++ch) {
             if (!first) __syncthreads();
@@ -307,9 +323,10 @@
 #pragma unroll
                     for (int rb = 0; rb < RB; ++rb)
 #pragma unroll
-                        for (int cg = 0; cg < YT; ++cg) {
-                            const bool valid = zx_ok && y0 + cg < p.H && (rb0 + rb) * 16 + 4 * g < p.M;
-                            mk[rb][cg] = __builtin_bit_cast(u32x2, vs_raw_buffer_load_b64(mrsrc, valid ? ebase + cg * p.W * p.M * 2 + rb * 32 : -1, 0, 0));
+                        for (int j = 0; j < NE; ++j) {
+                            const int cg = cgo + j;
+                            const bool valid = zx_ok && y0 + cg < p.H && (rbw + rb) * 16 + 4 * g < p.M;
+                            mk[rb][j] = __builtin_bit_cast(u32x2, vs_raw_buffer_load_b64(mrsrc, valid ? ebase + cg * p.W * p.M * 2 + rb * 32 : -1, 0, 0));
                         }
                 }
             }
@@ -323,20 +340,20 @@
             }
 
             K3_TICK(4);
-            auto read_kg = [&](int kg, u32x4 (&a)[RB], u32x4 (&b)[YT]) {
+            auto read_kg = [&](int kg, u32x4 (&a)[RB], u32x4 (&b)[NE]) {
 #pragma unroll
                 for (int rb = 0; rb < RB; ++rb) a[rb] = *(const u32x4*)(s_wl + (rb * NKGC + kg) * 1024);
                 if constexpr (SMALLC) {
                     const int o = baddr[0] + s_taps[kg * 4 + g];
 #pragma unroll
-                    for (int cg = 0; cg < YT; ++cg) b[cg] = *(const u32x4*)(s_tile + o + cg * 18 * CKB);
+                    for (int cg = 0; cg < NE; ++cg) b[cg] = *(const u32x4*)(s_tile + o + cg * 18 * CKB);
                 } else {
                     const int dz = kg / 9, dy = (kg / 3) % 3, dx = kg % 3;
 #pragma unroll
-                    for (int cg = 0; cg < YT; ++cg) b[cg] = *(const u32x4*)(s_tile + baddr[dx] + ((dz * PLANE + (dy + cg) * 18 + dx) * CKB));
+                    for (int cg = 0; cg < NE; ++cg) b[cg] = *(const u32x4*)(s_tile + baddr[dx] + ((dz * PLANE + (dy + cg) * 18 + dx) * CKB));
                 }
             };
-            u32x4 fa[2][RB], fb[2][YT];
+            u32x4 fa[2][RB], fb[2][NE];
             read_kg(0, fa[0], fb[0]);
 #pragma unroll
             for (int kg = 0; kg < NKGC; ++kg) {
@@ -344,7 +361,7 @@
 #pragma unroll
                 for (int rb = 0; rb < RB; ++rb)
 #pragma unroll
-                    for (int cg = 0; cg < YT; ++cg) acc[rb][cg] = mfma16(fa[kg & 1][rb], fb[kg & 1][cg], acc[rb][cg], (T*)nullptr);
+                    for (int cg = 0; cg < NE; ++cg) acc[rb][cg] = mfma16(fa[kg & 1][rb], fb[kg & 1][cg], acc[rb][cg], (T*)nullptr);
                 __builtin_amdgcn_sched_barrier(0);
             }
         }
@@ -372,32 +389,34 @@
                 }
             }
         } else {
+            float xs[CSPLIT ? RB : 1][CSPLIT ? NE : 1][4], xq[CSPLIT ? RB : 1][CSPLIT ? NE : 1][4];
 #pragma unroll
             for (int rb = 0; rb < RB; ++rb) {
-                const bool rvalid = (rb0 + rb) * 16 + 4 * g < p.M;
+                const bool rvalid = (rbw + rb) * 16 + 4 * g < p.M;
                 float mm[4] = {0.f, 0.f, 0.f, 0.f}, mr[4] = {0.f, 0.f, 0.f, 0.f};
                 if (has_sums && rvalid) {
-                    const int row = (rb0 + rb) * 16 + 4 * g;
+                    const int row = (rbw + rb) * 16 + 4 * g;
 #pragma unroll
                     for (int r = 0; r < 4; ++r) { mm[r] = s_mkm[n * p.M + row + r]; mr[r] = s_mkr[n * p.M + row + r]; }
                 }
 #pragma unroll
-                for (int cg = 0; cg < YT; ++cg) {
+                for (int j = 0; j < NE; ++j) {
+                    const int cg = cgo + j;
                     const bool valid = rvalid && zx_ok && y0 + cg < p.H;
                     f32x2 lo, hi;
-                    lo[0] = acc[rb][cg][0] + bv[rb][0]; lo[1] = acc[rb][cg][1] + bv[rb][1];
-                    hi[0] = acc[rb][cg][2] + bv[rb][2]; hi[1] = acc[rb][cg][3] + bv[rb][3];
+                    lo[0] = acc[rb][j][0] + bv[rb][0]; lo[1] = acc[rb][j][1] + bv[rb][1];
+                    hi[0] = acc[rb][j][2] + bv[rb][2]; hi[1] = acc[rb][j][3] + bv[rb][3];
                     i32x2 pk;
                     pk[0] = (int)H16<T>::pack2(lo);
                     pk[1] = (int)H16<T>::pack2(hi);
-                    if constexpr (EA) pkk[rb][cg] = pk;
+                    if constexpr (EA) pkk[rb][j] = pk;
                     else vs_raw_buffer_store_b64(pk, yrsrc, valid ? ebase + cg * p.W * p.M * 2 + rb * 32 : -1, 0, 0);
                     float v[4];
                     v[0] = H16<T>::lo((unsigned int)pk[0]); v[1] = H16<T>::hi((unsigned int)pk[0]);
                     v[2] = H16<T>::lo((unsigned int)pk[1]); v[3] = H16<T>::hi((unsigned int)pk[1]);
                     if (!valid) { v[0] = 0.f; v[1] = 0.f; v[2] = 0.f; v[3] = 0.f; }
                     if (has_sums) {
-                        const u32x2 xx = mk[rb][cg];
+                        const u32x2 xx = mk[rb][j];
                         float xv4[4];
                         xv4[0] = H16<T>::lo(xx[0]); xv4[1] = H16<T>::hi(xx[0]);
                         xv4[2] = H16<T>::lo(xx[1]); xv4[3] = H16<T>::hi(xx[1]);
@@ -405,16 +424,53 @@
                         for (int r = 0; r < 4; ++r) {
                             const float xh = (xv4[r] - mm[r]) * mr[r];
                             const float gm = xh > 0.f ? v[r] : 0.f;
-                            ssum[rb][r] += gm; ssq[rb][r] += gm * xh;
+                            if constexpr (CSPLIT) { xs[rb][j][r] = gm; xq[rb][j][r] = xh; }
+                            else { ssum[rb][r] += gm; ssq[rb][r] += gm * xh; }
                         }
                     } else {
 #pragma unroll
-                        for (int r = 0; r < 4; ++r) { ssum[rb][r] += v[r]; ssq[rb][r] += v[r] * v[r]; }
+                        for (int r = 0; r < 4; ++r) {
+                            if constexpr (CSPLIT) { xs[rb][j][r] = v[r]; xq[rb][j][r] = v[r]; }
+                            else { ssum[rb][r] += v[r]; ssq[rb][r] += v[r] * v[r]; }
+                        }
                     }
                 }
             }
             double* const red_dst0 = has_sums ? p.sums : p.y_stats;
             double* const red_dst = red_dst0;
+            if constexpr (CSPLIT) {
+                if (red_dst != nullptr) {
+                    float* s_x = (float*)(s_w + GEO::W_BYTES);
+                    auto xi = [&](int rb, int j, int r, int st) { return ((((wz * RB + rb) * NE + j) * 4 + r) * 2 + st) * 64 + lane; };
+                    if (q == 1) {
+#pragma unroll
+                        for (int rb = 0; rb < RB; ++rb)
+#pragma unroll
+                            for (int j = 0; j < NE; ++j)
+#pragma unroll
+                                for (int r = 0; r < 4; ++r) { s_x[xi(rb, j, r, 0)] = xs[rb][j][r]; s_x[xi(rb, j, r, 1)] = xq[rb][j][r]; }
+                    } else {
+#pragma unroll
+                        for (int rb = 0; rb < RB; ++rb)
+#pragma unroll
+                            for (int j = 0; j < NE; ++j)
+#pragma unroll
+                                for (int r = 0; r < 4; ++r) { ssum[rb][r] += xs[rb][j][r]; ssq[rb][r] += xs[rb][j][r] * xq[rb][j][r]; }
+                    }
+                    __syncthreads();
+                    if (q == 0) {
+#pragma unroll
+                        for (int rb = 0; rb < RB; ++rb)
+#pragma unroll
+                            for (int j = 0; j < NE; ++j)
+#pragma unroll
+                                for (int r = 0; r < 4; ++r) {
+                                    const float a = s_x[xi(rb, j, r, 0)], b = s_x[xi(rb, j, r, 1)];
+                                    ssum[rb][r] += a; ssq[rb][r] += a * b;
+                                }
+                    }
+                }
+            }
             if (red_dst != nullptr) {
                 const bool flush = t + G >= t_end || nxt.n != n;
                 if (flush) {
@@ -422,22 +478,23 @@
                     for (int rb = 0; rb < RB; ++rb)
 #pragma unroll
                         for (int r = 0; r < 4; ++r) {
-                            float s = ssum[rb][r], q = ssq[rb][r];
-                            { s = row16_sum(s); q = row16_sum(q); }
+                            float s = ssum[rb][r], sq = ssq[rb][r];
+                            { s = row16_sum(s); sq = row16_sum(sq); }
                             if (col == 0) {
-                                const int lr = rb * 16 + 4 * g + r;
-                                s_red[(wave * 64 + lr) * 2 + 0] = s;
-                                s_red[(wave * 64 + lr) * 2 + 1] = q;
+                                const int lr = (RPAIR ? q * MT : 0) + rb * 16 + 4 * g + r;
+                                s_red[(wave * RS + lr) * 2 + 0] = s;
+                                s_red[(wave * RS + lr) * 2 + 1] = sq;
                             }
                             ssum[rb][r] = 0.f; ssq[rb][r] = 0.f;
                         }
                     __syncthreads();
-                    if (tid < MT * 2) {
+                    if (tid < MTW * 2) {
                         const int lr = tid >> 1, st = tid & 1;
                         const int row = rb0 * 16 + lr;
                         if (row < p.M) {
-                            const double tot = (double)s_red[(0 * 64 + lr) * 2 + st] + (double)s_red[(1 * 64 + lr) * 2 + st] +
-                                               (double)s_red[(2 * 64 + lr) * 2 + st] + (double)s_red[(3 * 64 + lr) * 2 + st];
+                            const int w0 = RPAIR ? (lr / MT) * 4 : 0;
+                            const double tot = (double)s_red[((w0 + 0) * RS + lr) * 2 + st] + (double)s_red[((w0 + 1) * RS + lr) * 2 + st] +
+                                               (double)s_red[((w0 + 2) * RS + lr) * 2 + st] + (double)s_red[((w0 + 3) * RS + lr) * 2 + st];
                             stat_add(red_dst, (size_t)n * p.M + row, (size_t)p.N * p.M, st, tot);
                         }
                     }
@@ -448,7 +505,7 @@
                 unsigned int* ctr = p.ea_sync + (size_t)n * 256;
                 chain_arrive8(ctr);
                 chain_wait8(ctr, (unsigned int)p.ea_items, p.ea_fault);
-                if (tid < MT) {
+                if (tid < MTW) {
                     const int row = rb0 * 16 + tid;
                     float m = 0.f, r = 1.f, a = 0.f, b = 0.f;
                     if (row < p.M) {
@@ -463,15 +520,16 @@
                 __syncthreads();
 #pragma unroll
                 for (int rb = 0; rb < RB; ++rb) {
-                    const bool rvalid = (rb0 + rb) * 16 + 4 * g < p.M;
+                    const bool rvalid = (rbw + rb) * 16 + 4 * g < p.M;
                     f32x4 tb[4];
 #pragma unroll
-                    for (int r = 0; r < 4; ++r) tb[r] = *(const f32x4*)(s_red + (rb * 16 + 4 * g + r) * 4);
-#pragma unroll
-                    for (int cg = 0; cg < YT; ++cg) {
+                    for (int r = 0; r < 4; ++r) tb[r] = *(const f32x4*)(s_red + ((RPAIR ? q * MT : 0) + rb * 16 + 4 * g + r) * 4);
+#pragma unroll
+                    for (int j = 0; j < NE; ++j) {
+                        const int cg = cgo + j;
                         const bool valid = rvalid && zx_ok && y0 + cg < p.H;
-                        const unsigned int gw[2] = {(unsigned int)pkk[rb][cg][0], (unsigned int)pkk[rb][cg][1]};
-                        const u32x2 xx = mk[rb][cg];
+                        const unsigned int gw[2] = {(unsigned int)pkk[rb][j][0], (unsigned int)pkk[rb][j][1]};
+                        const u32x2 xx = mk[rb][j];
                         const float gv[4] = {H16<T>::lo(gw[0]), H16<T>::hi(gw[0]), H16<T>::lo(gw[1]), H16<T>::hi(gw[1])};
                         const float xq[4] = {H16<T>::lo(xx[0]), H16<T>::hi(xx[0]), H16<T>::lo(xx[1]), H16<T>::hi(xx[1])};
                         float o[4];
@@ -493,11 +551,44 @@
     K3_TICK_FLUSH;
 }
 
-static inline int k3b_ea_max_wgs(int n, int c, int m) {
-    using GEO = K3BGeom<32, 16, 4>;
-    const size_t lds = K3B_LDS_TILE + (size_t)GEO::TILE_BYTES + GEO::W_BYTES + (size_t)2 * n * c * sizeof(float) + (size_t)2 * n * m * sizeof(float);
-    return 2 * (lds + 1024) <= 160 * 1024 ? 512 : 256;
-}
+static inline int k3b_resident_wgs(const void* kern, int threads, size_t lds) {
+    struct Entry { const void* k; int dev; size_t lds; int wgs; };
+    static Entry cache[64];
+    static int used = 0;
+    static std::mutex mu;
+    int dev = 0;
+    if (hipGetDevice(&dev) != hipSuccess) return 0;
+    std::lock_guard<std::mutex> lock(mu);
+    for (int i = 0; i < used; ++i)
+        if (cache[i].k == kern && cache[i].dev == dev && cache[i].lds == lds) return cache[i].wgs;
+    int per_cu = 0, cus = 0;
+    if (hipOccupancyMaxActiveBlocksPerMultiprocessor(&per_cu, kern, threads, lds) != hipSuccess ||
+        hipDeviceGetAttribute(&cus, hipDeviceAttributeMultiprocessorCount, dev) != hipSuccess) return 0;
+    const int waves = (threads + 63) / 64;
+    const int max_per_cu = waves >= 24 ? 1 : 24 / waves;
+    if (per_cu > max_per_cu) per_cu = max_per_cu;
+    const int wgs = per_cu * cus;
+    if (used < 64) cache[used++] = Entry{kern, dev, lds, wgs};
+    return wgs;
+}
+
+template <typename T, int CK, int MT, int EPI, bool SUMS, int YT, bool HS, bool FA = false, bool EA = false, int NW = 4, int SPL = K3B_WAVES4>
+struct K3bInst {
+    using GEO = K3BGeom<CK, MT, YT, NW * 64, SPL == K3B_ROWS ? 2 : 1, SPL == K3B_COLS>;
+    static constexpr auto kern = k3b_kernel<CK, MT, EPI, SUMS, YT, HS, T, FA, EA, NW, SPL>;
+    static size_t lds(const G1Params& p) {
+        const size_t tables = (size_t)(FA ? 6 : 2) * p.N * p.C * sizeof(float) + (p.sums ? (size_t)2 * p.N * p.M * sizeof(float) : 0);
+        return K3B_LDS_TILE + (size_t)GEO::TILE_BYTES + GEO::W_BYTES + GEO::XS_BYTES + tables;
+    }
+    static hipError_t opt_in() {
+        static const hipError_t attr_err = hipFuncSetAttribute((const void*)kern, hipFuncAttributeMaxDynamicSharedMemorySize, 160 * 1024);
+        return attr_err;
+    }
+    static int capacity(const G1Params& p) {
+        if (opt_in() != hipSuccess) return 0;
+        return k3b_resident_wgs((const void*)kern, NW * 64, lds(p));
+    }
+};
 
 static inline void k3b_fastdiv(int d, unsigned int& m, unsigned int& s) {
     s = 0;
@@ -505,13 +596,16 @@
     m = (unsigned int)((((1ull << (32 + s)) + (unsigned long long)d - 1) / (unsigned long long)d) - (1ull << 32));
 }
 
-template <typename T, int CK, int MT, int EPI, bool SUMS, int YT, bool HS, bool FA = false, bool EA = false>
-static int k3b_launch_t(const G1Params& p_in, int tiles_total, int row_tiles, hipStream_t stream) {
-    using GEO = K3BGeom<CK, MT, YT>;
+template <typename T, int CK, int MT, int EPI, bool SUMS, int YT, bool HS, bool FA = false, bool EA = false, int NW = 4, int SPL = K3B_WAVES4>
+static int k3b_launch_t(const G1Params& p_in, int tiles_total, int row_tiles, hipStream_t stream, bool dry = false) {
+    using I = K3bInst<T, CK, MT, EPI, SUMS, YT, HS, FA, EA, NW, SPL>;
     if (FA && (p_in.N * p_in.C > 192 || (CK < 32 && p_in.nch != 1) || !p_in.x_stats || !p_in.fa_sums)) return VS_ESHAPE;
-    const size_t tables = (size_t)(FA ? 6 : 2) * p_in.N * p_in.C * sizeof(float) + (p_in.sums ? (size_t)2 * p_in.N * p_in.M * sizeof(float) : 0);
-    const size_t lds = K3B_LDS_TILE + (size_t)GEO::TILE_BYTES + GEO::W_BYTES + tables;
+    const size_t lds = I::lds(p_in);
     if (lds > 160 * 1024) return VS_ESHAPE;
+    if (SPL == K3B_ROWS) {
+        if (row_tiles % 2) return VS_ESHAPE;
+        row_tiles /= 2;
+    }
     G1Params p = p_in;
     if (YT != 4) {
         p.tyn = (p.H + YT - 1) / YT;
@@ -523,19 +617,19 @@
     k3b_fastdiv(p.txn * p.tyn, p.fd_m[1], p.fd_s[1]);
     k3b_fastdiv(p.txn, p.fd_m[2], p.fd_s[2]);
     if (SUMS != (p.sums != nullptr) || (SUMS && !FA && p.x_stats != nullptr)) return VS_EINVAL;
-    auto kern = k3b_kernel<CK, MT, EPI, SUMS, YT, HS, T, FA, EA>;
-    static const hipError_t attr_err =
-        hipFuncSetAttribute((const void*)kern, hipFuncAttributeMaxDynamicSharedMemorySize, 160 * 1024);
+    const hipError_t attr_err = I::opt_in();
     if (attr_err != hipSuccess) return (int)attr_err;
     const int per_cu = vs_cfg().k3_wgs_per_cu > 0 ? vs_cfg().k3_wgs_per_cu : 3;
     int wg = 256 * per_cu / (row_tiles < per_cu ? row_tiles : per_cu);
     if (wg < 256) wg = 256;
     const int gx = tiles_total < wg ? tiles_total : wg;
     if (EA) {
-        if (gx != tiles_total || (long long)tiles_total * row_tiles > k3b_ea_max_wgs(p.N, p.C, p.M) || !p.ea_sync || !p.ea_fault) return VS_ESHAPE;
+        if (gx != tiles_total || (long long)tiles_total * row_tiles > I::capacity(p)) return VS_ESHAPE;
+        if (!dry && (!p.ea_sync || !p.ea_fault)) return VS_ESHAPE;
         p.ea_items = p.tiles_per_sample * row_tiles;
     }
-    hipLaunchKernelGGL(kern, dim3(gx, row_tiles), dim3(256), lds, stream, p);
+    if (dry) return VS_OK;
+    hipLaunchKernelGGL(I::kern, dim3(gx, row_tiles), dim3(NW * 64), lds, stream, p);
     VS_CHECK_LAUNCH();
     return VS_OK;
 }
```

New measurement: 908.6 volumes/s, median of 6. 1.01x the previous value.
